# wgurecky/CORRLA_RS

Hardware: AMD Instinct MI355X
Metric: RSVD GFLOP/s on 16k x 16k f32 rank-128 (higher is better)
Workload: dtype f32

## Files before the change

corrla_rs_amd/_lib.py:

```python
import ctypes as C
import os

PKG = os.path.dirname(os.path.abspath(__file__))
LIB_PATH = os.environ.get("CORRLA_RSVD_LIB") or os.path.join(PKG, "lib", "libcorrla_rsvd.so")

i64, u64, u32, i32, dbl, flt = C.c_int64, C.c_uint64, C.c_uint32, C.c_int32, C.c_double, C.c_float
vp = C.c_void_p

OK, EINVAL, ENOMEM, EHIP, ECOMM, ENUMERIC, ENODEV = range(7)
OMEGA_ON_DEVICE = 0x1
PCA_CENTER_FUSED = 0x2
PCA_CENTER_COPY = 0x4
QR_HOUSEHOLDER = 0x8
SEED_EXPLICIT = 0x10
POWER_FUSED = 0x20
SHARD_COLS = 0x40
SKETCH_BF16X3 = 0x80
SKETCH_BF16X6 = 0x100
PCA_STANDARDIZE = 0x200
COV_CORRELATION = 0x1
COV_NO_CENTER = 0x2
COV_ROUTE_INPLACE, COV_ROUTE_INPLACE_CHECKED, COV_ROUTE_REPACKED = 1, 2, 3
COV_ROUTES = {COV_ROUTE_INPLACE: "inplace", COV_ROUTE_INPLACE_CHECKED: "inplace_checked", COV_ROUTE_REPACKED: "repacked"}
PCA_APPLY_OWN_MEANS = 0x400
PCA_APPLY_ROUTE_INPLACE, PCA_APPLY_ROUTE_INPLACE_CHECKED, PCA_APPLY_ROUTE_REPACKED = 1, 2, 3
PCA_APPLY_ROUTES = {PCA_APPLY_ROUTE_INPLACE: "inplace", PCA_APPLY_ROUTE_INPLACE_CHECKED: "inplace_checked",
                    PCA_APPLY_ROUTE_REPACKED: "repacked"}
PCA_APPLY_CENTRINGS = {1: "fused", 2: "copy"}
UNIQUE_ID_BYTES = 128


class Opts(C.Structure):
    _fields_ = [("struct_size", u32), ("flags", u32), ("seed", u64), ("omega", vp), ("omega_ld", i64),
                ("scales_out", vp)]


class Timings(C.Structure):
    _fields_ = [("total_ms", dbl), ("sketch_ms", dbl), ("power_ms", dbl), ("qr_ms", dbl), ("project_ms", dbl),
                ("small_svd_ms", dbl), ("finalize_ms", dbl), ("qr_passes", i32), ("n_collectives", i32),
                ("sketch_kernel_ms", dbl), ("host_enqueue_ms", dbl), ("collective_bytes", dbl), ("n_mixed_products", i32),
                ("n_bf16_products", i32), ("knn_ms", dbl), ("fit_ms", dbl)]


def _sigs():
    s = {
        "corrla_version": (C.c_char_p, []),
        "corrla_last_error": (C.c_char_p, []),
        "corrla_device_count": (C.c_int, []),
        "corrla_ctx_create": (C.c_int, [C.c_int, C.POINTER(vp)]),
        "corrla_ctx_destroy": (None, [vp]),
        "corrla_ctx_synchronize": (C.c_int, [vp]),
        "corrla_ctx_get_timings": (C.c_int, [vp, C.POINTER(Timings)]),
        "corrla_ctx_set_phase_timings": (C.c_int, [vp, C.c_int]),
        "corrla_ctx_comm_info": (C.c_int, [vp, C.POINTER(C.c_int), C.POINTER(C.c_int)]),
        "corrla_comm_unique_id": (C.c_int, [vp]),
        "corrla_ctx_comm_init": (C.c_int, [vp, vp, C.c_int, C.c_int]),
        "corrla_ctx_last_pca_apply": (C.c_int, [vp, C.POINTER(C.c_int), C.POINTER(C.c_int)]),
    }
    for suf, sc in (("f32", flt), ("f64", dbl)):
        rsvd = [vp, vp, i64, i64, i64, i64, i64, i64, i64, C.POINTER(Opts), vp, i64, vp, vp, i64]
        s["corrla_rsvd_" + suf] = (C.c_int, rsvd)
        s["corrla_rsvd_dev_" + suf] = (C.c_int, rsvd)
        s["corrla_rsvd_sharded_dev_" + suf] = (C.c_int, rsvd)
        pca = [vp, vp, i64, i64, i64, i64, i64, i64, i64, C.POINTER(Opts), vp, vp, vp, i64]
        s["corrla_pca_" + suf] = (C.c_int, pca)
        s["corrla_pca_dev_" + suf] = (C.c_int, pca)
        s["corrla_pca_sharded_dev_" + suf] = (C.c_int, pca)
        pw = [vp, vp, i64, i64, i64, i64, i64, i64, C.POINTER(Opts), vp, i64]
        s["corrla_power_iter_" + suf] = (C.c_int, pw)
        s["corrla_power_iter_dev_" + suf] = (C.c_int, pw)
        s["corrla_matmul_dev_" + suf] = (C.c_int, [vp, C.c_int, vp, i64, i64, i64, i64, vp, i64, i64, sc, vp, i64])
        rsvd_csr = [vp, vp, vp, vp, i64, i64, i64, i64, i64, i64, C.POINTER(Opts), vp, i64, vp, vp, i64]
        s["corrla_rsvd_csr_" + suf] = (C.c_int, rsvd_csr)
        s["corrla_rsvd_csr_dev_" + suf] = (C.c_int, rsvd_csr)
        pca_csr = [vp, vp, vp, vp, i64, i64, i64, i64, i64, i64, C.POINTER(Opts), vp, vp, vp, i64]
        s["corrla_pca_csr_" + suf] = (C.c_int, pca_csr)
        s["corrla_pca_csr_dev_" + suf] = (C.c_int, pca_csr)
        s["corrla_spmm_csr_dev_" + suf] = (C.c_int, [vp, C.c_int, vp, vp, vp, i64, i64, i64, vp, i64, i64, sc, vp, i64])
        cov = [vp, vp, i64, i64, i64, i64, u64, C.c_int, vp, vp, vp, i64, C.POINTER(C.c_int)]
        s["corrla_cov_" + suf] = (C.c_int, cov)
        s["corrla_cov_dev_" + suf] = (C.c_int, cov)
        model = [vp, vp, vp, i64, i64, u64, vp, i64, vp, vp]
        s["corrla_pca_transform_" + suf] = s["corrla_pca_transform_dev_" + suf] = (C.c_int, [vp, vp, i64, i64, i64, i64] + model)
        s["corrla_pca_transform_csr_" + suf] = s["corrla_pca_transform_csr_dev_" + suf] = (C.c_int, [vp, vp, vp, vp, i64, i64, i64] + model)
        inverse = [vp, vp, i64, i64, i64, vp, vp, vp, i64, i64, vp, i64]
        s["corrla_pca_inverse_" + suf] = s["corrla_pca_inverse_dev_" + suf] = (C.c_int, inverse)
        points = [vp, vp, i64, i64, vp, i64, i64, i64, C.c_int, dbl]
        s["corrla_rbf_matrix_" + suf] = s["corrla_rbf_matrix_dev_" + suf] = (C.c_int, points + [vp, i64])
        s["corrla_rbf_apply_" + suf] = s["corrla_rbf_apply_dev_" + suf] = (C.c_int, points + [C.c_int, vp, i64, i64, vp, i64])
        s["corrla_fill_normal_dev_" + suf] =(C.c_int, [vp, vp, i64, i64, i64, i64, u64, i64, i64])
        s["corrla_time_sketch_dev_" + suf] = (C.c_int, [vp, vp, i64, i64, i64, i64, vp, i64, i64, vp, i64, C.c_int,
                                                         C.POINTER(dbl)])
    s["corrla_rsvd_bf16"] = s["corrla_rsvd_dev_bf16"] = s["corrla_rsvd_f32"]
    s["corrla_pca_bf16"] = s["corrla_pca_dev_bf16"] = s["corrla_pca_f32"]
    s["corrla_matmul_dev_bf16"] = s["corrla_matmul_dev_f32"]
    grad = [vp, vp, i64, i64, vp, vp, i64, C.c_int, i64, dbl, vp, i64, C.POINTER(C.c_int)]
    s["corrla_grad_mat_f64"] = (C.c_int, grad)
    s["corrla_grad_mat_dev_f64"] = (C.c_int, grad)
    return s


SIGNATURES = _sigs()
_lib = None


class CorrlaError(RuntimeError):
    def __init__(self, code, msg):
        super().__init__(f"corrla_rsvd error {code}: {msg}")
        self.code = code


def load():
    global _lib
    if _lib is not None:
        return _lib
    if not os.path.exists(LIB_PATH):
        raise ImportError(
            f"{LIB_PATH} is missing: build it with `python -m corrla_rs_amd.build` (hipcc, gfx950). "
            "corrla_rs_amd has no CPU fallback.")
    try:
        import torch
    except ImportError:
        pass
    lib = C.CDLL(LIB_PATH, mode=C.RTLD_GLOBAL)
    for name, (res, args) in SIGNATURES.items():
        fn = getattr(lib, name)
        fn.restype = res
        fn.argtypes = args
    _lib = lib
    return lib


def check(code):
    if code != OK:
        msg = load().corrla_last_error().decode("utf-8", "replace")
        if code == EINVAL:
            raise ValueError(f"corrla_rsvd: {msg}")
        if code == ENOMEM:
            raise MemoryError(f"corrla_rsvd: {msg}")
        raise CorrlaError(code, msg)
```

corrla_rs_amd/api.py:

```python
import atexit
import ctypes as C
import sys
import threading
import weakref

import numpy as np

from . import _lib as L

__all__ = ["Context", "default_context", "rsvd", "random_svd", "power_iter", "rpca", "PcaRsvd", "algorithmic_flops"]


def _is_torch(x):
    return type(x).__module__.split(".")[0] == "torch"


def _is_torch_csr(x):
    return _is_torch(x) and str(getattr(x, "layout", "")) == "torch.sparse_csr"


def _is_sparse(x):
    if isinstance(x, tuple):
        def nd(v):
            return v.ndim if hasattr(v, "ndim") else np.ndim(v)
# ... 549 lines not shown
        if on_dev:
            import torch
            out = torch.empty((n_q, n_s), dtype=xq.dtype, device=xq.device)
            _sync_stream(xq)
        else:
            out = np.empty((n_q, n_s), dtype=xq.dtype)
        L.check(self._entry("corrla_rbf_matrix_", on_dev, xq.dtype)(self._h, _ptr(xq), n_q, self._row_stride(xq), _ptr(xs), n_s,
                                                                   self._row_stride(xs), dim, self._rbf_kernel_id(kernel_type),
                                                                   float(kernel_param), _ptr(out), n_s))
        if on_dev:
            L.check(self._lib.corrla_ctx_synchronize(self._h))
        return out

    def rbf_apply(self, x_query, x_support, coeffs, kernel_type, kernel_param=0.0, *, poly_degree=None):
        xq, xs, on_dev = self._rbf_points(x_query, x_support, "rbf_apply")
        n_q, dim = (int(v) for v in xq.shape)
        n_s = int(xs.shape[0])
        if poly_degree is not None and (isinstance(poly_degree, (bool, np.bool_)) or not isinstance(poly_degree, (int, np.integer))):
            raise ValueError("poly_degree must be None or an integer")
        degree = -1 if poly_degree is None or poly_degree < 0 else int(poly_degree)
        n_poly = 0 if degree < 0 else (dim + 1 if degree < 2 else dim + dim * (dim + 1) // 2 + 1)
        _reject_bf16(coeffs, "rbf_apply")
        if _is_sparse(coeffs):
            raise ValueError("rbf_apply takes dense coefficients")
        w = self._model_array(coeffs, xq, on_dev)
        if w.ndim == 1:
            w = w.reshape(-1, 1)
        if w.ndim != 2 or w.shape[1] == 0:
            raise ValueError("coeffs must be a non-empty matrix")
        if w.shape[0] != n_s + n_poly:
            raise ValueError(f"coeffs must have n_s + n_poly = {n_s} + {n_poly} rows, got {w.shape[0]}")
        w = self._rbf_rowmajor(w, on_dev)
        n_rhs = int(w.shape[1])
        if on_dev:
            import torch
            out = torch.empty((n_q, n_rhs), dtype=xq.dtype, device=xq.device)
            _sync_stream(xq)
        else:
            out = np.empty((n_q, n_rhs), dtype=xq.dtype)
        L.check(self._entry("corrla_rbf_apply_", on_dev, xq.dtype)(self._h, _ptr(xq), n_q, self._row_stride(xq), _ptr(xs), n_s,
                                                                  self._row_stride(xs), dim, self._rbf_kernel_id(kernel_type),
                                                                  float(kernel_param), degree, _ptr(w), self._row_stride(w), n_rhs,
                                                                  _ptr(out), n_rhs))
        if on_dev:
            L.check(self._lib.corrla_ctx_synchronize(self._h))
        return out

    def _run_product(self, name, operand, m, n, xt, trans, beta, in_dtype=None):
        import torch
        xin, xout = (m, n) if trans else (n, m)
        l = xt.shape[1]
        xc = xt.t().contiguous()
        res = torch.empty((l, xout), dtype=xt.dtype, device=xt.device)
        _sync_stream(xt)
        L.check(self._entry(name, True, in_dtype or xt.dtype)(self._h, 1 if trans else 0, *_c_args(operand), xc.data_ptr(), xin, l, float(beta),
                                                  res.data_ptr(), xout))
        return res.t()

    def spmm(self, a_csr, x, trans=False, beta=1.0):
        import torch
        vals, ci, rp, (m, n), on_dev = _as_csr(a_csr)
        dev = torch.device(f"cuda:{self.device}")
        if not on_dev:
            vals, ci, rp = (torch.from_numpy(v).to(dev) for v in (vals, ci, rp))
        xt = x if _is_torch(x) else torch.as_tensor(np.asarray(x))
        xt = xt.to(device=dev, dtype=vals.dtype)
        if xt.dim() != 2 or xt.shape[0] != (m if trans else n):
            raise ValueError(f"x must have {m if trans else n} rows")
        return self._run_product("corrla_spmm_csr_", (vals, ci, rp, m, n, int(vals.shape[0])),
                                 m, n, xt, trans, beta)

    def matmul(self, a, x, trans=False, beta=1.0):
        m, n = a.shape
        if _is_bf16(x):
            raise ValueError("matmul: x must be float32 or float64 (only the matrix a may be bfloat16)")
        if _is_bf16(a):
            if not str(x.dtype).endswith("float32"):
                raise ValueError("matmul: a bfloat16 a takes a float32 x")
            assert x.shape[0] == (m if trans else n)
            return self._run_product("corrla_matmul_", (a, m, n, *a.stride()), m, n, x, trans, beta, in_dtype=a.dtype)
        assert x.shape[0] == (m if trans else n) and x.dtype == a.dtype
        return self._run_product("corrla_matmul_", (a, m, n, *a.stride()), m, n, x, trans, beta)

    def grad_mat(self, x_mat, y, est_order, n_nbrs, x_query=None, *, scale=1.0):
        est_order, n_nbrs = int(est_order), int(n_nbrs)
        nreg = C.c_int(0)
        if _is_torch(x_mat) and x_mat.is_cuda:
            import torch
            x = x_mat.to(torch.float64).contiguous()
            yv = (y if _is_torch(y) else torch.as_tensor(np.asarray(y))).to(device=x.device, dtype=torch.float64).reshape(-1).contiguous()
            xq = x if x_query is None else x_query.to(device=x.device, dtype=torch.float64).contiguous()
            if x.dim() != 2 or xq.dim() != 2 or xq.shape[1] != x.shape[1] or yv.numel() != x.shape[0]:
                raise ValueError("x_mat (n, k), y (n,), x_query (n_q, k) expected")
            g = torch.empty((xq.shape[0], x.shape[1]), dtype=torch.float64, device=x.device)
            _sync_stream(x)
            L.check(self._lib.corrla_grad_mat_dev_f64(self._h, x.data_ptr(), x.shape[0], x.shape[1], yv.data_ptr(), xq.data_ptr(),
                                                      xq.shape[0], est_order, n_nbrs, float(scale), g.data_ptr(), x.shape[1],
                                                      C.byref(nreg)))
            return g.t(), nreg.value
        x = np.ascontiguousarray(np.asarray(x_mat, dtype=np.float64))
        yv = np.ascontiguousarray(np.asarray(y, dtype=np.float64).reshape(-1))
        xq = x if x_query is None else np.ascontiguousarray(np.asarray(x_query, dtype=np.float64))
        if x.ndim != 2 or xq.ndim != 2 or xq.shape[1] != x.shape[1] or yv.size != x.shape[0]:
            raise ValueError("x_mat (n, k), y (n,), x_query (n_q, k) expected")
        g = np.empty((xq.shape[0], x.shape[1]), dtype=np.float64)
        L.check(self._lib.corrla_grad_mat_f64(self._h, x.ctypes.data, x.shape[0], x.shape[1], yv.ctypes.data, xq.ctypes.data,
                                              xq.shape[0], est_order, n_nbrs, float(scale), g.ctypes.data, x.shape[1],
                                              C.byref(nreg)))
        return g.T, nreg.value

    def power_iter(self, a_mat, omega_rank, n_iter, *, seed=None, omega=None, qr=None):
        _reject_bf16(a_mat, "power_iter")
        a = np.asarray(a_mat)
        if a.ndim != 2:
            raise ValueError("a_mat must be 2-D")
        if a.dtype != np.float32:
            a = a.astype(np.float64, copy=False)
        m, n = a.shape
        w = int(omega_rank)
        rs, cs = _strides(a)
        o, keep = self._opts(seed, omega, n, w, a.dtype, False, self._qr_flag(qr))
        q = _empty_colmajor(a, m, max(w, 1))
        fn = self._entry("corrla_power_iter_", False, a.dtype)
        L.check(fn(self._h, a.ctypes.data, m, n, rs, cs, w, int(n_iter), C.byref(o) if o is not None else None,
                   q.ctypes.data, m))
        del keep
        return q

    def fill_normal(self, t, seed, row0=0, global_cols=None):
        rows, cols = t.shape
        rs, cs = t.stride()
        _sync_stream(t)
        fn = self._entry("corrla_fill_normal_", True, t.dtype)
        L.check(fn(self._h, t.data_ptr(), rows, cols, rs, cs, int(seed), int(row0),
                   int(global_cols if global_cols is not None else cols)))
        return t

    def time_sketch(self, a, x, reps=10):
        import torch
        m, n = a.shape
        rs, cs = a.stride()
        l = x.shape[1]
        xc = x.t().contiguous()
        y = torch.empty((l, m), dtype=a.dtype, device=a.device)
        ms = C.c_double()
        _sync_stream(a)
        fn = self._entry("corrla_time_sketch_", True, a.dtype)
        L.check(fn(self._h, a.data_ptr(), m, n, rs, cs, xc.data_ptr(), n, l, y.data_ptr(), m, int(reps), C.byref(ms)))
        return ms.value, y.t()


_default = None
_default_lock = threading.Lock()


def default_context():
    global _default
    with _default_lock:
        if _default is None:
            _default = Context(0)
        return _default


def rsvd(a_mat, n_rank, n_iters, n_oversamples, *, seed=None, omega=None, ctx=None, qr=None):
    return (ctx or default_context()).rsvd(a_mat, n_rank, n_iters, n_oversamples, seed=seed, omega=omega, qr=qr)

# ... 87 lines not shown
```

corrla_rs_amd/csrc/capi_impl.hpp:

```cpp
#pragma once
#include <cstddef>
#include <cstdint>
#include <cstring>
#include <string>
#include <vector>

#include "../../include/corrla_rsvd.h"
#include "driver.hpp"
#include "rbf_plan.hpp"

namespace corrla {

inline std::string& last_error_slot() {
  static thread_local std::string msg;
  return msg;
}

template <class F>
inline corrla_status guarded(F&& f) {
  try {
    f();
    return CORRLA_OK;
  } catch (const Error& e) {
    last_error_slot() = e.what();
// ... 368 lines not shown
    if (scales_out) dev.copy_values_out(sd.p, c.n, scales_out, c.host_ptrs);
  });
  finish_call(drv, dev, c.tm_out, false);
}

template <class Dev, class T>
inline void pca_entry(Dev& dev, bool host_ptrs, const T* x, int64_t m, int64_t n, int64_t rs, int64_t cs, int64_t rank,
                      int64_t n_iter, int64_t n_oversamples, const corrla_opts* opts, T* means, T* s, T* comps,
                      int64_t ldc, Timings* tm_out, bool profile, bool sharded = false) {
  PcaCall<T> c{host_ptrs, m, n, rank, n_iter, n_oversamples, opts, means, s, comps, ldc, tm_out, profile};
  c.sharded = sharded;
  pca_body(
      dev, c,
      [&] {
        validate_matrix(x, m, n, rs, cs);
        if (sharded) {
          if (rank < 1 || rank > n) throw Error(ST_EINVAL, "rank must be in [1, n_dim] for the sample-sharded PCA");
          if (n_iter < 0 || n_oversamples < 0) throw Error(ST_EINVAL, "n_iter and n_oversamples must be >= 0");
        } else {
          validate_rank(m, n, rank, n_iter, n_oversamples);
        }
      },
      [&] { return stage_input<Dev, T>(dev, host_ptrs, x, m, n, rs, cs, sharded); });
}

template <class Dev, class T>
inline void power_iter_entry(Dev& dev, bool host_ptrs, const T* a, int64_t m, int64_t n, int64_t rs, int64_t cs,
                             int64_t width, int64_t n_iter, const corrla_opts* opts, T* q, int64_t ldq) {
  if (!q) throw Error(ST_EINVAL, "q is NULL");
  validate_matrix(a, m, n, rs, cs);
  if (width < 1 || width > n) throw Error(ST_EINVAL, "width must be in [1, n]");
  if (n_iter < 0) throw Error(ST_EINVAL, "n_iter must be >= 0");
  if (ldq < m) throw Error(ST_EINVAL, "ldq < m");
  RunOpts ro = parse_opts(opts, !host_ptrs);
  if (ro.omega && ro.omega_ld < n) throw Error(ST_EINVAL, "omega_ld < n");
  if (!ro.seed_explicit && !ro.omega) ro.seed = dev.fresh_seed(false);
  dev.begin_call();
  TallA<T> ta = stage_input<Dev, T>(dev, host_ptrs, a, m, n, rs, cs, true);
  RsvdDriver<Dev, T> drv(dev, false);
  Skinny<T> y = dev.template alloc_skinny<T>(ta.mt, width);
  Skinny<T> y2 = dev.template alloc_skinny<T>(ta.mt, width);
  drv.power_iter(ta, width, n_iter, ro, y, y2);
  dev.copy_out(y, width, q, ldq, false, host_ptrs);
  dev.end_call();
}

template <class Dev, class T, class Validate, class Stage>
inline void product_body(Dev& dev, int trans, int64_t m, int64_t n, const T* x, int64_t ldx, int64_t l, T beta, T* res,
                         int64_t ldres, Timings* tm_out, Validate&& validate, Stage&& stage) {
  if (!x || !res) throw Error(ST_EINVAL, "x or res is NULL");
  validate();
  if (l < 1) throw Error(ST_EINVAL, "l must be >= 1");
  const int64_t xin = trans ? m : n, xout = trans ? n : m;
  if (ldx < xin || ldres < xout) throw Error(ST_EINVAL, "leading dimension too small");
  dev.begin_call();
  TallA<T> ta = stage();
  RsvdDriver<Dev, T> drv(dev, false);
  if (!ta.sparse) drv.mixed_planes_ = parse_opts(nullptr, true).mixed_planes;
  Skinny<T> xs = dev.template alloc_skinny<T>(xin, l);
  dev.copy_in_skinny(x, ldx, xs);
  Skinny<T> out = ta.sparse ? caller_skinny(res, xout, l, ldres) : dev.template alloc_skinny<T>(xout, l);
  T* beta_dev = dev.template alloc_scalar<T>(1);
  dev.store_values(&beta, (int64_t)1, beta_dev, false);
  if (trans)
    drv.at_times(ta, xs, out, beta_dev, false);
  else
    drv.a_times(ta, xs, out, beta_dev);
  if (!out.external) dev.copy_out(out, l, res, ldres, false, false);
  dev.end_call();
  if (tm_out) {
    tm_out->n_mixed_products = drv.tm.n_mixed_products;
    tm_out->n_bf16_products = drv.tm.n_bf16_products;
  }
}

template <class Dev, class T>
inline void matmul_entry(Dev& dev, int trans, const T* a, int64_t m, int64_t n, int64_t rs, int64_t cs, const T* x,
                         int64_t ldx, int64_t l, T beta, T* res, int64_t ldres, Timings* tm_out = nullptr) {
  product_body(
      dev, trans, m, n, x, ldx, l, beta, res, ldres, tm_out, [&] { validate_matrix(a, m, n, rs, cs); },
      [&] { return stage_input<Dev, T>(dev, false, a, m, n, rs, cs, true); });
}

inline void validate_csr_args(const void* values, const void* ci, const void* rp, int64_t m, int64_t n, int64_t nnz) {
  if (!values || !ci || !rp) throw Error(ST_EINVAL, "values, col_idx or row_ptr is NULL");
  if (m < 1 || n < 1) throw Error(ST_EINVAL, "matrix must have at least one row and one column");
  if (m > 0x7fffffff || n > 0x7fffffff) throw Error(ST_EINVAL, "CSR input: m and n must be below 2^31");
  if (nnz < 1) throw Error(ST_EINVAL, "CSR input: nnz must be >= 1");
  if (nnz > 0x7fffffff) throw Error(ST_EINVAL, "CSR input: nnz must be below 2^31");
}

template <class Dev, class T>
inline TallA<T> stage_csr(Dev& dev, bool host_ptrs, const T* values, const int32_t* ci, const int64_t* rp, int64_t m, int64_t n,
                          int64_t nnz, bool keep_orientation) {
  CsrView<T> a;
  a.rows = m;
  a.cols = n;
  a.nnz = nnz;
  if (host_ptrs) {
    if (rp[m] != nnz) throw Error(ST_EINVAL, "invalid CSR matrix: row_ptr[m] != nnz");
    T* dv = (T*)dev.alloc_bytes(sizeof(T) * (size_t)nnz);
    int32_t* dc = (int32_t*)dev.alloc_bytes(sizeof(int32_t) * (size_t)nnz);
    int64_t* dr = (int64_t*)dev.alloc_bytes(sizeof(int64_t) * (size_t)(m + 1));
    dev.h2d_bytes(dv, values, sizeof(T) * (size_t)nnz);
    dev.h2d_bytes(dc, ci, sizeof(int32_t) * (size_t)nnz);
    dev.h2d_bytes(dr, rp, sizeof(int64_t) * (size_t)(m + 1));
    a.val = dv;
    a.ci = dc;
    a.rp = dr;
  } else {
    a.val = values;
    a.ci = ci;
    a.rp = rp;
  }
  dev.csr_plan(a, true);
  CsrView<T> at = dev.csr_transpose(a);
  dev.csr_plan(at, false);
  TallA<T> ta;
  ta.sparse = true;
  const bool fat = !keep_orientation && m < n;
  ta.mt = fat ? n : m;
  ta.nt = fat ? m : n;
  ta.csr = fat ? at : a;
  ta.csr_t = fat ? a : at;
  return ta;
}

template <class Dev, class T>
inline void rsvd_csr_entry(Dev& dev, bool host_ptrs, const T* values, const int32_t* ci, const int64_t* rp, int64_t m, int64_t n,
                           int64_t nnz, int64_t rank, int64_t n_iter, int64_t n_oversamples, const corrla_opts* opts, T* u,
                           int64_t ldu, T* s, T* vt, int64_t ldvt, Timings* tm_out, bool profile) {
  static_assert(dev_has_spmm<Dev>::value, "CSR entries need a backend with SpMM kernels");
  RsvdCall<T> c{host_ptrs, m, rank, n_iter, n_oversamples, opts, u, ldu, s, vt, ldvt, tm_out, profile};
  c.sparse = true;
  c.fat = m < n;
  rsvd_body(
      dev, c,
      [&] {
        validate_csr_args(values, ci, rp, m, n, nnz);
        validate_rank(m, n, rank, n_iter, n_oversamples);
      },
      [&] { return stage_csr<Dev, T>(dev, host_ptrs, values, ci, rp, m, n, nnz, false); });
}

template <class Dev, class T>
inline void pca_csr_entry(Dev& dev, bool host_ptrs, const T* values, const int32_t* ci, const int64_t* rp, int64_t m, int64_t n,
                          int64_t nnz, int64_t rank, int64_t n_iter, int64_t n_oversamples, const corrla_opts* opts, T* means,
                          T* s, T* comps, int64_t ldc, Timings* tm_out, bool profile) {
  static_assert(dev_has_spmm<Dev>::value, "CSR entries need a backend with SpMM kernels");
  PcaCall<T> c{host_ptrs, m, n, rank, n_iter, n_oversamples, opts, means, s, comps, ldc, tm_out, profile};
  c.sparse = true;
  pca_body(
      dev, c,
      [&] {
        validate_csr_args(values, ci, rp, m, n, nnz);
        validate_rank(m, n, rank, n_iter, n_oversamples);
      },
      [&] { return stage_csr<Dev, T>(dev, host_ptrs, values, ci, rp, m, n, nnz, false); });
}

template <class Dev, class T>
inline void spmm_entry(Dev& dev, int trans, const T* values, const int32_t* ci, const int64_t* rp, int64_t m, int64_t n, int64_t nnz,
                       const T* x, int64_t ldx, int64_t l, T beta, T* res, int64_t ldres) {
  static_assert(dev_has_spmm<Dev>::value, "CSR entries need a backend with SpMM kernels");
  product_body(
      dev, trans, m, n, x, ldx, l, beta, res, ldres, (Timings*)nullptr, [&] { validate_csr_args(values, ci, rp, m, n, nnz); },
// ... 276 lines not shown
```

corrla_rs_amd/csrc/corrla_rsvd.hip:

```cpp
#include <mutex>
#include <vector>

#include "capi_impl.hpp"
#include "core_svd_stage.hpp"
#include "cov_stage.hpp"
#include "grad_stage.hpp"
#include "hip_backend.hpp"
#include "pca_apply_stage.hpp"
#include "rbf_stage.hpp"
#include "tall_stage.hpp"

using namespace corrla;

struct corrla_ctx {
  HipDev dev;
  Timings last;
  std::mutex mu;
  bool profile;
  pca_apply_stage::Ran pca_apply;
  explicit corrla_ctx(int ordinal) : dev(ordinal), profile(env_int("CORRLA_PROFILE_PHASES", 0) != 0) {}
};

namespace {
inline corrla_ctx* need(corrla_ctx* c) {
  if (!c) throw Error(ST_EINVAL, "ctx is NULL");
  return c;
}
template <class F>
inline void locked_call(corrla_ctx* c, F&& f) {
  std::lock_guard<std::mutex> lk(c->mu);
  try {
    f();
  } catch (...) {
    (void)hipSetDevice(c->dev.device);
    if (c->dev.stream) (void)hipStreamSynchronize(c->dev.stream);
    (void)hipGetLastError();
    throw;
  }
}

template <class F, class After>
inline corrla_status ctx_call(corrla_ctx* ctx, F&& f, After&& after) {
  return guarded([&] {
    corrla_ctx* c = need(ctx);
    locked_call(c, [&] { f(*c); });
    after(*c);
  });
}
template <class F>
inline corrla_status ctx_call(corrla_ctx* ctx, F&& f) {
  return ctx_call(ctx, f, [](corrla_ctx&) {});
}
inline void debug_qr_breakdown(const corrla_ctx& c) {
  if (c.profile && env_int("CORRLA_DEBUG", 0))
    std::fprintf(stderr, "[corrla] qr breakdown (ms): gram %.3f  download+check %.3f  host chol/inv %.3f  upload+apply %.3f  (%d passes)\n",
                 c.last.qr_gram_ms, c.last.qr_down_ms, c.last.qr_host_ms, c.last.qr_apply_ms, c.last.qr_passes);
}
template <class T>
corrla_status fill_c(corrla_ctx* ctx, T* p, int64_t rows, int64_t cols, int64_t rs, int64_t cs, uint64_t seed,
                     int64_t row0, int64_t global_cols) {
  return guarded([&] {
    corrla_ctx* c = need(ctx);
    if (!p) throw Error(ST_EINVAL, "p is NULL");
    if (rows < 0 || cols < 0 || rs < 0 || cs < 0 || global_cols < cols) throw Error(ST_EINVAL, "bad fill_normal shape");
    std::lock_guard<std::mutex> lk(c->mu);
    CORRLA_HIP(hipSetDevice(c->dev.device));
    c->dev.fill_normal(p, rows, cols, rs, cs, seed, row0, global_cols);
    c->dev.sync();
  });
}
template <class T>
corrla_status time_sketch_c(corrla_ctx* ctx, const T* a, int64_t m, int64_t n, int64_t rs, int64_t cs, const T* x,
                            int64_t ldx, int64_t l, T* y, int64_t ldy, int reps, double* avg_ms) {
  return guarded([&] {
    corrla_ctx* c = need(ctx);
    if (!x || !y || !avg_ms) throw Error(ST_EINVAL, "NULL argument");
    if (reps < 1 || l < 1 || ldx < n || ldy < m) throw Error(ST_EINVAL, "bad time_sketch arguments");
    std::lock_guard<std::mutex> lk(c->mu);
    HipDev& dev = c->dev;
    dev.begin_call();
    TallA<T> ta = stage_input<HipDev, T>(dev, false, a, m, n, rs, cs, true);
    RsvdDriver<HipDev, T> drv(dev, false);
    drv.mixed_planes_ = parse_opts(nullptr, true).mixed_planes;
    Skinny<T> xs = dev.alloc_skinny<T>(n, l);
    dev.copy_in_skinny(x, ldx, xs);
    Skinny<T> out = dev.alloc_skinny<T>(m, l);
    *avg_ms = dev.time_on_stream(reps, [&] { drv.a_times(ta, xs, out, nullptr); });
    dev.copy_out(out, l, y, ldy, false, false);
    dev.end_call();
  });
}
}

// ... 156 lines not shown
      pca_bf16_entry<HipDev>(c.dev, HOST, x, m, n, rs, cs, rank, n_iter, p, o, means, s, comps, ldc, &c.last, c.profile); \
    });                                                                                                                 \
  }
CORRLA_DEFINE_RSVD_BF16(corrla_rsvd_bf16, true)
CORRLA_DEFINE_RSVD_BF16(corrla_rsvd_dev_bf16, false)
CORRLA_DEFINE_PCA_BF16(corrla_pca_bf16, true)
CORRLA_DEFINE_PCA_BF16(corrla_pca_dev_bf16, false)
CORRLA_API corrla_status corrla_matmul_dev_bf16(corrla_ctx* ctx, int trans, CORRLA_DENSE(uint16_t, a), CORRLA_PRODUCT_REST(float)) {
  return ctx_call(ctx, [&](corrla_ctx& c) {
    matmul_bf16_entry<HipDev>(c.dev, trans, a, m, n, rs, cs, x, ldx, l, beta, res, ldres, &c.last);
  });
}

#define CORRLA_DEFINE_COV(NAME, T, HOST)                                                                                \
  CORRLA_API corrla_status NAME(corrla_ctx* ctx, CORRLA_DENSE(T, x), uint64_t flags, int ddof, T* means_out, T* scales_out, \
                                T* c, int64_t ldc, int* route_out) {                                                    \
    return ctx_call(ctx, [&](corrla_ctx& cx) {                                                                          \
      cov_entry<HipDev, T>(cx.dev, x, m, n, rs, cs, flags, ddof, means_out, scales_out, c, ldc, route_out, [&] {        \
        cov_stage::run<T>(cx.dev, HOST, x, m, n, rs, cs, flags, ddof, means_out, scales_out, c, ldc, route_out);        \
      });                                                                                                               \
    });                                                                                                                 \
  }
CORRLA_DEFINE_COV(corrla_cov_f32, float, true)
CORRLA_DEFINE_COV(corrla_cov_f64, double, true)
CORRLA_DEFINE_COV(corrla_cov_dev_f32, float, false)
CORRLA_DEFINE_COV(corrla_cov_dev_f64, double, false)

#define CORRLA_PCA_MODEL(T) const T *means, const T *scales, const T *components, int64_t ldc, int64_t k, uint64_t flags, T *scores, \
                            int64_t ld_scores, T *resid_out, T *means_out
#define CORRLA_PCA_MODEL_CALL(T) PcaTransformCall<T>{m, n, means, scales, components, ldc, k, flags, scores, ld_scores, resid_out, means_out}
#define CORRLA_DEFINE_PCA_TRANSFORM(NAME, T, HOST)                                                                      \
  CORRLA_API corrla_status NAME(corrla_ctx* ctx, CORRLA_DENSE(T, x), CORRLA_PCA_MODEL(T)) {                             \
    return ctx_call(ctx, [&](corrla_ctx& cx) {                                                                          \
      cx.pca_apply = pca_apply_stage::Ran();                                                                            \
      const PcaTransformCall<T> c = CORRLA_PCA_MODEL_CALL(T);                                                           \
      if (!x) throw Error(ST_EINVAL, "pca_transform: x is NULL");                                                       \
      if (m < 1 || n < 1) throw Error(ST_EINVAL, "pca_transform: m and n must be >= 1");                                \
      if (rs < 0 || cs < 0) throw Error(ST_EINVAL, "pca_transform: negative strides are not supported");                \
      const PcaApplyRange xr{x, (size_t)((m - 1) * rs + (n - 1) * cs + 1) * sizeof(T), "x"};                            \
      pca_transform_entry<HipDev, T>(cx.dev, c, false, &xr, 1,                                                          \
                                     [&] { pca_apply_stage::run_dense<T>(cx.dev, HOST, x, rs, cs, c, &cx.pca_apply); }); \
    });                                                                                                                 \
  }
#define CORRLA_DEFINE_PCA_TRANSFORM_CSR(NAME, T, HOST)                                                                  \
  CORRLA_API corrla_status NAME(corrla_ctx* ctx, CORRLA_CSR_A(T), CORRLA_PCA_MODEL(T)) {                                \
    return ctx_call(ctx, [&](corrla_ctx& cx) {                                                                          \
      cx.pca_apply = pca_apply_stage::Ran();                                                                            \
      const PcaTransformCall<T> c = CORRLA_PCA_MODEL_CALL(T);                                                           \
      validate_csr_args(values, col_idx, row_ptr, m, n, nnz);                                                           \
      const PcaApplyRange op[3] = {{values, (size_t)nnz * sizeof(T), "values"},                                         \
                                   {col_idx, (size_t)nnz * sizeof(int32_t), "col_idx"},                                 \
                                   {row_ptr, (size_t)(m + 1) * sizeof(int64_t), "row_ptr"}};                            \
      pca_transform_entry<HipDev, T>(cx.dev, c, true, op, 3, [&] {                                                      \
        pca_apply_stage::run_csr<T>(cx.dev, HOST, values, col_idx, row_ptr, nnz, c, &cx.pca_apply);                     \
      });                                                                                                               \
    });                                                                                                                 \
  }
#define CORRLA_DEFINE_PCA_INVERSE(NAME, T, HOST)                                                                        \
  CORRLA_API corrla_status NAME(corrla_ctx* ctx, const T* scores, int64_t m, int64_t k, int64_t ld_scores, const T* means, \
                                const T* scales, const T* components, int64_t ldc, int64_t n, T* out, int64_t row_stride_out) { \
    return ctx_call(ctx, [&](corrla_ctx& cx) {                                                                          \
      cx.pca_apply = pca_apply_stage::Ran();                                                                            \
      pca_inverse_entry<HipDev, T>(cx.dev, scores, m, k, ld_scores, means, scales, components, ldc, n, out, row_stride_out, [&] { \
        pca_apply_stage::run_inverse<T>(cx.dev, HOST, scores, m, k, ld_scores, means, scales, components, ldc, n, out,   \
                                        row_stride_out, &cx.pca_apply);                                                 \
      });                                                                                                               \
    });                                                                                                                 \
  }
#define CORRLA_DEFINE_PCA_APPLY(SUF, T)                                  \
  CORRLA_DEFINE_PCA_TRANSFORM(corrla_pca_transform_##SUF, T, true)       \
  CORRLA_DEFINE_PCA_TRANSFORM(corrla_pca_transform_dev_##SUF, T, false)  \
  CORRLA_DEFINE_PCA_TRANSFORM_CSR(corrla_pca_transform_csr_##SUF, T, true)      \
  CORRLA_DEFINE_PCA_TRANSFORM_CSR(corrla_pca_transform_csr_dev_##SUF, T, false) \
  CORRLA_DEFINE_PCA_INVERSE(corrla_pca_inverse_##SUF, T, true)           \
  CORRLA_DEFINE_PCA_INVERSE(corrla_pca_inverse_dev_##SUF, T, false)
CORRLA_DEFINE_PCA_APPLY(f32, float)
CORRLA_DEFINE_PCA_APPLY(f64, double)
CORRLA_API corrla_status corrla_ctx_last_pca_apply(corrla_ctx* ctx, int* centring_out, int* route_out) {
  return guarded([&] {
    corrla_ctx* c = need(ctx);
    std::lock_guard<std::mutex> lk(c->mu);
    if (centring_out) *centring_out = c->pca_apply.centring;
    if (route_out) *route_out = c->pca_apply.route;
  });
}

#define CORRLA_RBF_POINTS(T) const T *xq, int64_t n_q, int64_t ldq, const T *xs, int64_t n_s, int64_t lds, int64_t dim, int kernel, double eps
#define CORRLA_DEFINE_RBF(SUF, DEV, T, HOST)                                                                            \
  CORRLA_API corrla_status corrla_rbf_matrix_##DEV##SUF(corrla_ctx* ctx, CORRLA_RBF_POINTS(T), T* out, int64_t ld_out) { \
    return ctx_call(ctx, [&](corrla_ctx& cx) {                                                                          \
      const RbfCall<T> c{xq, n_q, ldq, xs, n_s, lds, dim, kernel, eps, -1, nullptr, 0, 0, out, ld_out};                 \
      rbf_matrix_entry<HipDev, T>(cx.dev, c, [&] { rbf_stage::run_matrix<T>(cx.dev, HOST, c); });                       \
    });                                                                                                                 \
  }                                                                                                                     \
  CORRLA_API corrla_status corrla_rbf_apply_##DEV##SUF(corrla_ctx* ctx, CORRLA_RBF_POINTS(T), int poly_degree, const T* coeffs, \
                                                       int64_t ldw, int64_t n_rhs, T* out, int64_t ld_out) {            \
    return ctx_call(ctx, [&](corrla_ctx& cx) {                                                                          \
      const RbfCall<T> c{xq, n_q, ldq, xs, n_s, lds, dim, kernel, eps, poly_degree, coeffs, ldw, n_rhs, out, ld_out};   \
      rbf_apply_entry<HipDev, T>(cx.dev, c, [&] { rbf_stage::run_apply<T>(cx.dev, HOST, c); });                         \
    });                                                                                                                 \
  }
CORRLA_DEFINE_RBF(f32, , float, true)
CORRLA_DEFINE_RBF(f64, , double, true)
CORRLA_DEFINE_RBF(f32, dev_, float, false)
CORRLA_DEFINE_RBF(f64, dev_, double, false)

static corrla_status grad_mat_c(corrla_ctx* ctx, bool host_ptrs, const double* x, int64_t n_pts, int64_t kf, const double* y,
                                const double* xq, int64_t n_q, int est_order, int64_t n_nbrs, double out_scale, double* g,
                                int64_t ldg, int* n_regularised) {
  return ctx_call(ctx, [&](corrla_ctx& c) {
    HipDev& dev = c.dev;
    if (!x || !y || !xq || !g) throw Error(ST_EINVAL, "NULL argument");
    if (n_pts < 1 || n_q < 1 || kf < 1) throw Error(ST_EINVAL, "empty point set");
    if (ldg < kf) throw Error(ST_EINVAL, "ldg < k");
    const GradPlan plan = grad_plan(n_pts, kf, n_q, est_order, n_nbrs, env_int("CORRLA_KNN", 0), env_int("CORRLA_FIT", 0),
                                    dev.num_cus, kGradWideBudgetBytes, env_int("CORRLA_KNN2_WGS_PER_CU", 1));
    if (plan.error) throw Error(ST_EINVAL, plan.error);
    dev.begin_call();
    auto dbl = [&](int64_t n) { return (double*)dev.alloc_bytes(sizeof(double) * (size_t)n); };
    auto staged = [&](const double* h, int64_t n) {
      if (!host_ptrs) return h;
      double* d = dbl(n);
      CORRLA_HIP(hipMemcpyAsync(d, h, sizeof(double) * (size_t)n, hipMemcpyHostToDevice, dev.stream));
      return (const double*)d;
    };
    const GradCall call{staged(x, n_pts * kf), staged(y, n_pts), staged(xq, n_q * kf), host_ptrs ? dbl(n_q * kf) : g,
                        host_ptrs ? kf : ldg, n_pts, kf, n_q, n_nbrs, est_order, out_scale,
                        (int*)dev.alloc_bytes(sizeof(int) * (size_t)(n_q * n_nbrs)), (int*)dev.alloc_bytes(sizeof(int) * (size_t)n_q),
                        env_int("CORRLA_KNN2_PROF", 0) != 0};
    grad_stage::run(dev, call, plan);
    std::vector<int> hs((size_t)n_q);
    CORRLA_HIP(hipMemcpyAsync(hs.data(), call.status, sizeof(int) * (size_t)n_q, hipMemcpyDeviceToHost, dev.stream));
    if (host_ptrs)
      CORRLA_HIP(hipMemcpy2DAsync(g, sizeof(double) * (size_t)ldg, call.g, sizeof(double) * (size_t)kf, sizeof(double) * (size_t)kf,
                                  (size_t)n_q, hipMemcpyDeviceToHost, dev.stream));
    dev.event_mark(2);
    dev.end_call();
    c.last = Timings();
    c.last.knn_ms = dev.event_elapsed_ms(0, 1);
    c.last.fit_ms = dev.event_elapsed_ms(1, 2);
    c.last.total_ms = c.last.knn_ms + c.last.fit_ms;
    int bad = 0;
    for (int v : hs) bad += v != 0;
    if (n_regularised) *n_regularised = bad;
  });
}
CORRLA_API corrla_status corrla_grad_mat_f64(corrla_ctx* ctx, const double* x, int64_t n_pts, int64_t k, const double* y,
                                             const double* xq, int64_t n_q, int est_order, int64_t n_nbrs, double out_scale,
                                             double* g, int64_t ldg, int* n_regularised) {
  return grad_mat_c(ctx, true, x, n_pts, k, y, xq, n_q, est_order, n_nbrs, out_scale, g, ldg, n_regularised);
}
CORRLA_API corrla_status corrla_grad_mat_dev_f64(corrla_ctx* ctx, const double* x, int64_t n_pts, int64_t k, const double* y,
                                                 const double* xq, int64_t n_q, int est_order, int64_t n_nbrs,
                                                 double out_scale, double* g, int64_t ldg, int* n_regularised) {
  return grad_mat_c(ctx, false, x, n_pts, k, y, xq, n_q, est_order, n_nbrs, out_scale, g, ldg, n_regularised);
}

CORRLA_API corrla_status corrla_comm_unique_id(void* out128) {
  return guarded([&] {
    if (!out128) throw Error(ST_EINVAL, "out128 is NULL");
    ncclUniqueId id;
    CORRLA_NCCL(ncclGetUniqueId(&id));
    std::memset(out128, 0, CORRLA_UNIQUE_ID_BYTES);
    std::memcpy(out128, &id, sizeof(id));
  });
}
// ... 11 lines not shown
```

corrla_rs_amd/csrc/driver.hpp:

```cpp
#pragma once
#include <cstdio>
#include <chrono>
#include <cmath>
#include <cstdint>
#include <cstring>
#include <limits>
#include <stdexcept>
#include <string>
#include <functional>
#include <type_traits>
#include <vector>

#include "gemm_plan.hpp"
#include "small_linalg.hpp"

namespace corrla {

struct Error : std::runtime_error {
  int code;
  Error(int c, const std::string& m) : std::runtime_error(m), code(c) {}
};
enum { ST_OK = 0, ST_EINVAL = 1, ST_ENOMEM = 2, ST_EHIP = 3, ST_ECOMM = 4, ST_ENUMERIC = 5, ST_ENODEV = 6 };

inline int64_t round_up(int64_t x, int64_t a) { return (x + a - 1) / a * a; }


template <class T>
struct Skinny {
  T* p = nullptr;
  int64_t rows = 0, cols = 0, ld = 0, cols_alloc = 0;
  bool external = false;
  Skinny view_cols(int64_t c) const {
    Skinny s = *this;
    s.cols = c;
    return s;
  }
};

template <class T>
struct Big {
  const T* p = nullptr;
  int64_t rows = 0, cols = 0, ld = 0, cols_readable = 0;
};

template <class T>
inline Big<T> as_rowmajor_transposed(const Skinny<T>& y, int64_t ncols) {
  Big<T> b;
  b.p = y.p;
  b.rows = ncols;
  b.cols = y.rows;
  b.ld = y.ld;
  b.cols_readable = y.ld;
  return b;
}

template <class T>
struct CsrView {
  const T* val = nullptr;
  const int32_t* ci = nullptr;
  const int64_t* rp = nullptr;
  int64_t rows = 0, cols = 0, nnz = 0;
  int64_t n_long = 0, n_chunks = 0;
  const int64_t* long_row = nullptr;
  const int64_t* long_base = nullptr;
  const int32_t* chunk_long = nullptr;
};

template <class D, class = void>
struct dev_has_spmm : std::false_type {};
template <class D>
struct dev_has_spmm<D, std::void_t<decltype(D::kHasSpmm)>> : std::true_type {};

template <class D, class = void>
struct dev_has_bf16in : std::false_type {};
template <class D>
struct dev_has_bf16in<D, std::void_t<decltype(D::kHasBf16In)>> : std::true_type {};

template <class D, class = void>
struct dev_has_colvar : std::false_type {};
template <class D>
struct dev_has_colvar<D, std::void_t<decltype(D::kHasColVar)>> : std::true_type {};

template <class D, class = void>
struct dev_has_syrk : std::false_type {};
template <class D>
struct dev_has_syrk<D, std::void_t<decltype(D::kHasSyrk)>> : std::true_type {};

template <class D, class = void>
struct dev_has_pca_apply : std::false_type {};
template <class D>
struct dev_has_pca_apply<D, std::void_t<decltype(D::kHasPcaApply)>> : std::true_type {};

template <class D, class = void>
struct dev_has_rbf : std::false_type {};
template <class D>
struct dev_has_rbf<D, std::void_t<decltype(D::kHasRbf)>> : std::true_type {};

template <class T>
struct TallA {
  Big<T> mem;
  bool row_major = true;
  int64_t mt = 0, nt = 0;
  const T* mu_short = nullptr;
  const T* mu_tall = nullptr;
  const T* inv_sd_short = nullptr;
  const T* inv_sd_tall = nullptr;
  bool sparse = false;
  CsrView<T> csr, csr_t;
  bool bf16 = false;
  Big<uint16_t> mem16;
};

struct RunOpts {
  uint64_t seed = 0x5eedull;
  bool seed_explicit = false;
  const void* omega = nullptr;
  int64_t omega_ld = 0;
  bool omega_on_device = false;
  bool sharded = false;
  int pca_center = 0;
  bool pca_standardize = false;
  bool qr_householder = false;
  bool power_fused = false;
  int mixed_planes = 0;
  bool mixed_project = true;
  int poison_core = 0;
};
constexpr int kFlagNonFinite = 2, kFlagNullCols = 4;

struct Timings {
  double total_ms = 0, sketch_ms = 0, power_ms = 0, qr_ms = 0, project_ms = 0, small_svd_ms = 0, finalize_ms = 0;
  double host_enqueue_ms = 0;
  int qr_passes = 0;
  int n_collectives = 0;
  double collective_bytes = 0;
  double knn_ms = 0, fit_ms = 0;
  int n_mixed_products = 0;
  int n_bf16_products = 0;
  double qr_gram_ms = 0, qr_down_ms = 0, qr_host_ms = 0, qr_apply_ms = 0;
  double sketch_kernel_ms = 0;
};

struct PhaseTimer {
  using clk = std::chrono::steady_clock;
  clk::time_point t0;
  PhaseTimer() : t0(clk::now()) {}
  double lap() {
    auto t1 = clk::now();
    double ms = std::chrono::duration<double, std::milli>(t1 - t0).count();
    t0 = t1;
    return ms;
  }
};

template <class Dev, class T>
struct RsvdDriver {
  Dev& dev;
  Timings tm;
  bool profile_phases;
  bool qr_householder = false;
  static constexpr const T* kNone = nullptr;

  explicit RsvdDriver(Dev& d, bool profile = false) : dev(d), profile_phases(profile) {}

  int mixed_planes_ = 0;
  void sparse_times(const CsrView<T>& s, const Skinny<T>& x, Skinny<T>& y, const T* scale_dev) {
    if constexpr (dev_has_spmm<Dev>::value)
      dev.spmm(s, x, y, scale_dev);
    else
      throw Error(ST_EINVAL, "this backend has no SpMM kernels: sparse operands are not supported");
  }
  void bf16_times(bool tn, const Big<uint16_t>& r, const Skinny<T>& x, Skinny<T>& y, const T* scale_dev) {
    if constexpr (dev_has_bf16in<Dev>::value && std::is_same<T, float>::value)
      dev.gemm_bf16a(tn, r, x, y, scale_dev), ++tm.n_bf16_products;
    else
      throw Error(ST_EINVAL, "this backend has no bf16-input kernels: bf16 operands are not supported");
  }
  Skinny<T> scale_ws_;
  void set_scale_workspace(const Skinny<T>& ws) { scale_ws_ = ws; }
// ... 85 lines not shown
    }
  };
  struct Attempt {
    bool defer = false;
    void* st_pool = nullptr;
    int st_slots = 0, st_used = 0;
    int* flags_pool = nullptr;
    int flags_cap = 0, flags_used = 0;
    std::vector<Pending> pending;
    bool dirty = false;
  } att_;
  void* status_record(int i) const { return (char*)att_.st_pool + (size_t)i * kStatusBytes; }
  int64_t m_local_ = 0, m_global_ = -1;
  int64_t m_local_override_ = -1;
  int64_t global_rows(bool sharded) {
    if (!sharded) return m_local_;
    if (m_global_ < 0) m_global_ = dev.allreduce_sum_host(m_local_);
    return m_global_;
  }

  int hh_short_shards_ = -1;
  bool householder_usable(const Skinny<T>& y, bool sharded) {
    if (!qr_householder) return false;
    if (!sharded) return y.rows >= y.cols;
    if (hh_short_shards_ < 0) hh_short_shards_ = (int)dev.allreduce_sum_host(m_local_ < y.cols ? 1 : 0);
    return hh_short_shards_ == 0;
  }
  void householder_panel(Skinny<T>& y, Skinny<T>& tmp, bool sharded) {
    const int64_t l = y.cols;
    auto h = dev.householder_up(y, tmp);
    if (!sharded) {
      dev.householder_down(h, y, tmp);
      return;
    }
    const int64_t np = dev.nranks(), rk = dev.rank();
    Skinny<T> stack = dev.template alloc_skinny<T>(np * l, l), t2 = dev.template alloc_skinny<T>(np * l, l);
    Skinny<T> rv, cv;
    rv.p = h.r_root();
    rv.rows = rv.cols = rv.ld = rv.cols_alloc = l;
    dev.copy_block(rv, 0, 0, l, l, stack, rk * l, 0);
    dev.allreduce(stack.p, (size_t)stack.ld * (size_t)stack.cols_alloc);
    dev.householder_thin_q(stack, t2);
    cv.p = (T*)dev.alloc_zeroed_bytes((size_t)l * (size_t)l * sizeof(T));
    cv.rows = cv.cols = cv.ld = cv.cols_alloc = l;
    dev.copy_block(stack, rk * l, 0, l, l, cv, 0, 0);
    dev.householder_down(h, y, tmp, (const T*)cv.p);
  }
  void householder_thin_q_any_width(Skinny<T>& y, Skinny<T>& tmp, bool sharded) {
    const int64_t l = y.cols, m = y.rows;
    int64_t wmax = dev.template householder_max_width<T>();
    if (const char* e = std::getenv("CORRLA_HH_BLOCK")) wmax = std::max<int64_t>(1, std::min<int64_t>(wmax, std::atoll(e)));
    if (l <= wmax) {
      householder_panel(y, tmp, sharded);
      return;
    }
    const int64_t nb = (l + wmax - 1) / wmax, w = (l + nb - 1) / nb;
    std::vector<double> th;
    for (int64_t c0 = 0; c0 < l; c0 += w) {
      const int64_t wb = std::min(w, l - c0);
      Skinny<T> yb = dev.template alloc_skinny<T>(m, wb), tb = dev.template alloc_skinny<T>(m, wb);
      Skinny<T> pb = dev.template alloc_skinny<T>(m, wb);
      dev.copy_block(y, 0, c0, m, wb, yb, 0, 0);
      for (int pass = 0; pass < 5; ++pass) {
        double overlap2 = 0.0;
        if (c0 > 0) {
          Skinny<T> t = dev.template alloc_skinny<T>(c0, wb);
          dev.gemm_nn(as_rowmajor_transposed(y, c0), yb, t, kNone);
          if (sharded) dev.allreduce(t.p, (size_t)t.ld * (size_t)t.cols_alloc);
          if (pass >= 1) {
            th.resize((size_t)(c0 * wb));
            dev.download_skinny(t, c0, wb, th.data());
            for (double v : th) overlap2 += v * v;
          }
          dev.gemm_tn(as_rowmajor_transposed(y, c0), t, pb, kNone);
          dev.sub_inplace(yb, pb);
        }
        householder_panel(yb, tb, sharded);
        if (c0 == 0 || (pass >= 1 && overlap2 <= 0.25)) break;
      }
      dev.copy_block(yb, 0, 0, m, wb, y, 0, c0);
    }
  }

  int64_t orthonormalize(Skinny<T>& y, Skinny<T>& tmp, bool sharded, bool rough = false) {
    const int64_t l = y.cols;
    if (householder_usable(y, sharded)) {
      PhaseTimer qt0;
      householder_thin_q_any_width(y, tmp, sharded);
      ++tm.qr_passes;
      subphase(tm.qr_gram_ms, qt0);
      return l;
    }
    int64_t r = orthonormalize_core(y, tmp, sharded, rough);
    if (r < l && !att_.defer && (sharded ? global_rows(true) : y.rows) >= l) r = complete_basis(y, r, sharded);
    return r;
  }

  int64_t complete_basis(Skinny<T>& y, int64_t r, bool sharded) {
    const int64_t l = y.cols, c = l - r, m = y.rows;
    Skinny<T> yc = dev.template alloc_skinny<T>(m, c);
    Skinny<T> pc = dev.template alloc_skinny<T>(m, c);
    Skinny<T> tc = dev.template alloc_skinny<T>(m, c);
    dev.fill_normal(yc.p, m, c, (int64_t)1, yc.ld, (uint64_t)(0x9e3779b97f4a7c15ull ^ (uint64_t)(131 * r + l)), (int64_t)0, c);
    if (r > 0) {
      for (int pass = 0; pass < 2; ++pass) {
        Skinny<T> t = dev.template alloc_skinny<T>(r, c);
        dev.gemm_nn(as_rowmajor_transposed(y, r), yc, t, kNone);
        if (sharded) dev.allreduce(t.p, (size_t)t.ld * (size_t)t.cols_alloc);
        dev.gemm_tn(as_rowmajor_transposed(y, r), t, pc, kNone);
        dev.sub_inplace(yc, pc);
      }
    }
    const int64_t rc = orthonormalize_core(yc, tc, sharded, false);
    dev.copy_cols(yc, y, r, rc);
    return r + rc;
  }

  template <class Factor>
  void cholqr_pass(Skinny<T>& y, Skinny<T>& tmp, Skinny<T>& gd, bool sharded, bool inplace, Factor&& factor) {
    const int64_t l = y.cols;
    Skinny<T> yv = y.view_cols(l);
    dev.gemm_nn(as_rowmajor_transposed(y, l), yv, gd, kNone);
    if (sharded) dev.allreduce(gd.p, (size_t)gd.ld * (size_t)gd.cols_alloc);
    const Skinny<T> md = factor(gd);
    if (inplace) {
      dev.apply_inplace(y, l, md);
    } else {
      dev.gemm_tn(as_rowmajor_transposed(y, l), md, tmp, kNone);
      std::swap(y.p, tmp.p);
    }
  }

  struct BlockSplit {
    int64_t n1 = 0, n2 = 0;
    T* minus_one = nullptr;
  };
  BlockSplit block_split(int64_t l) {
    BlockSplit s;
    s.n1 = round_up((l + 1) / 2, (int64_t)4);
    s.n2 = l - s.n1;
    s.minus_one = dev.template alloc_scalar<T>(1);
    dev.fill_const(s.minus_one, (int64_t)1, (T)-1);
    return s;
  }
  template <class Factor>
  void blocked_factor_inverse(const Skinny<T>& g, const BlockSplit& s, Skinny<T>& md, Factor&& factor) {
    const int64_t n1 = s.n1, n2 = s.n2;
    Skinny<T> g11 = dev.template alloc_skinny<T>(n1, n1), g12 = dev.template alloc_skinny<T>(n1, n2);
    Skinny<T> g22 = dev.template alloc_skinny<T>(n2, n2), x11 = dev.template alloc_skinny<T>(n1, n1);
    Skinny<T> x22 = dev.template alloc_skinny<T>(n2, n2), r12 = dev.template alloc_skinny<T>(n1, n2);
    Skinny<T> t22 = dev.template alloc_skinny<T>(n2, n2), t12 = dev.template alloc_skinny<T>(n1, n2);
    Skinny<T> x12 = dev.template alloc_skinny<T>(n1, n2);
    dev.copy_block(g, 0, 0, n1, n1, g11, 0, 0);
    dev.copy_block(g, 0, n1, n1, n2, g12, 0, 0);
    dev.copy_block(g, n1, n1, n2, n2, g22, 0, 0);
    factor(g11, n1, 0, x11);
    dev.gemm_nn(as_rowmajor_transposed(x11, n1), g12, r12, kNone);
    dev.gemm_nn(as_rowmajor_transposed(r12, n2), r12, t22, kNone);
    dev.sub_inplace(g22, t22);
    factor(g22, n2, 1, x22);
    dev.gemm_tn(as_rowmajor_transposed(r12, n2), x22, t12, kNone);
    dev.gemm_tn(as_rowmajor_transposed(x11, n1), t12, x12, s.minus_one);
    dev.copy_block(x11, 0, 0, n1, n1, md, 0, 0);
    dev.copy_block(x12, 0, 0, n1, n2, md, 0, n1);
    dev.copy_block(x22, 0, 0, n2, n2, md, n1, n1);
  }

  int64_t orthonormalize_device(Skinny<T>& y, Skinny<T>& tmp, bool sharded, bool rough, bool polish) {
    const int64_t l = y.cols;
    PhaseTimer qt0;
    const bool inplace = dev.qr_inplace_fits(l);
    const bool single = dev.template device_chol_fits<T>(l);
    const int level = std::max(2, std::min(dev.robust_passes(), kRobustPasses));
    const bool inloop = rough && !polish;
    const int npass_even = level;
    const int npass = inloop ? (level <= 2 ? 1 : npass_even - 1) : (polish ? (level <= 2 ? 1 : 3) : level);
    const int always = (polish || inloop) ? 1 : 2;
    int* need = att_.flags_pool + att_.flags_used;
    int* null_mask = dev.alloc_flags((int)l);
    int* need_blk = dev.alloc_flags(2);
    void* st_scratch = dev.alloc_zeroed_bytes((size_t)2 * npass * kStatusBytes);
    void* insp = single ? nullptr : dev.template alloc_inspect<T>();
    Skinny<T> gd = dev.template alloc_skinny<T>(l, l);
    Skinny<T> md = dev.template alloc_skinny<T>(l, l);
    const double eps0 = (double)std::numeric_limits<T>::epsilon();
    double shift_rel = eps0 * std::max({16.0, 0.25 * std::sqrt((double)std::max<int64_t>(y.rows, 1)), single ? 0.0 : 2.0 * (double)l});
    if (const char* e = std::getenv("CORRLA_QR_SHIFT_SCALE")) shift_rel *= std::atof(e);
    float nullx = 1.f;
    if (const char* e = std::getenv("CORRLA_QR_NULL_EXCESS")) nullx = (float)std::atof(e);
    const BlockSplit split = single ? BlockSplit{} : block_split(l);
    for (int pass = 0; pass < npass; ++pass) {
      const int gate = pass < always ? -1 : (inplace ? pass - 1 : always + ((pass - always) / 2) * 2 - 1);
      dev.set_run_if(gate < 0 ? nullptr : need + gate);
      const int shift_mode = polish ? 2 : (pass == 0 ? 1 : 0);
      const float nx = (!polish && pass >= 2) ? nullx : 0.f;
      const float need_ratio = (inloop && pass == 0) ? 1e-2f : 0.f;
      cholqr_pass(y, tmp, gd, sharded, inplace, [&](Skinny<T>& g) {
        if (single) {
          dev.chol_inv_robust(g, l, kPivotTol, (float)shift_rel, shift_mode, nx, md, st_scratch, pass, need + pass, null_mask, nullptr,
                              need_ratio);
          return md;
        }
        dev.gram_inspect(g, l, (float)shift_rel, shift_mode, insp);
        const void* shp = dev.template inspect_shift_ptr<T>(insp);
        blocked_factor_inverse(g, split, md, [&](const Skinny<T>& blk, int64_t n, int which, Skinny<T>& x) {
          dev.chol_inv_robust(blk, n, kPivotTol, 0.f, 2, nx, x, st_scratch, 2 * pass + which, need_blk + which,
                              null_mask + which * split.n1, shp, need_ratio);
        });
        dev.template combine_need<T>(need + pass, need_ratio > 0.f ? nullptr : insp, need_blk, need_blk + 1);
        return md;
      });
      if (pass + 1 < npass || inloop)
        dev.refill_null(y, l, null_mask, (uint64_t)(0x9e3779b97f4a7c15ull ^ (uint64_t)(977 * (att_.flags_used + pass) + l)));
      if (pass < always) ++tm.qr_passes;
    }
    dev.set_run_if(nullptr);
    att_.pending.push_back(Pending::robust_chol(always, npass, (inloop && npass > 1) ? -1 : att_.flags_used, st_scratch, single ? 1 : 2));
    att_.flags_used += npass;
    subphase(tm.qr_gram_ms, qt0);
    return l;
  }

  int64_t orthonormalize_core(Skinny<T>& y, Skinny<T>& tmp, bool sharded, bool rough, bool polish = false) {
    const int64_t l = y.cols;
    int64_t r = l;
    if (att_.defer && (sharded || y.rows >= l) && att_.flags_used + kRobustPasses <= att_.flags_cap &&
        dev.template device_qr_robust_fits<T>(l))
      return orthonormalize_device(y, tmp, sharded, rough, polish);
    const int rpp = dev.template device_chol_fits<T>(l) ? 1 : (dev.template device_chol_blocked_fits<T>(l) ? 2 : 0);
    if (rpp > 0) {
      PhaseTimer qt0;
      const int npass = rough ? 1 : 2, nrec = npass * rpp;
      Skinny<T> gd0 = dev.template alloc_skinny<T>(l, l);
      Skinny<T> md0 = rpp == 1 ? dev.template alloc_skinny<T>(l, l) : Skinny<T>{};
      const bool defer = att_.defer && att_.st_used + nrec <= att_.st_slots;
      void* st_dev = defer ? status_record(att_.st_used) : dev.alloc_bytes((size_t)2 * rpp * kStatusBytes);
      const BlockSplit split = rpp == 1 ? BlockSplit{} : block_split(l);
      for (int pass = 0; pass < npass; ++pass) {
        cholqr_pass(y, tmp, gd0, sharded, false, [&](Skinny<T>& g) {
          if (rpp == 1) {
            dev.chol_inv(g, l, kPivotTol, md0, st_dev, pass);
            return md0;
          }
          Skinny<T> md = dev.template alloc_skinny<T>(l, l);
          blocked_factor_inverse(g, split, md, [&](const Skinny<T>& blk, int64_t n, int which, Skinny<T>& x) {
            dev.chol_inv(blk, n, kPivotTol, x, st_dev, 2 * pass + which);
          });
          return md;
        });
        ++tm.qr_passes;
      }
      if (defer) {
        att_.pending.push_back(Pending::optimistic_chol(att_.st_used, npass, rpp, !rough));
        att_.st_used += nrec;
        subphase(tm.qr_gram_ms, qt0);
        return l;
      }
      int fail[4] = {0, 0, 0, 0};
      float min_ratio[4], dev_i[4];
      dev.read_chol_status(st_dev, nrec, fail, min_ratio, dev_i);
      subphase(tm.qr_gram_ms, qt0);
      bool ok = true;
      for (int i = 0; i < nrec; ++i) {
        if (fail[i] == 3) throw Error(ST_ENUMERIC, "non-finite Gram matrix in orthonormalisation");
        ok = ok && fail[i] == 0;
      }
      if (rpp == 1 && fail[0] == 2) return 0;
      for (int i = nrec - rpp; !rough && i < nrec; ++i) ok = ok && dev_i[i] <= 0.25f;
      if (ok) return l;
    }
    if (att_.defer) att_.dirty = true;
    const double eps = (double)std::numeric_limits<T>::epsilon();
    std::vector<double> g((size_t)l * l), mm((size_t)l * l), uu, ss, vv;
    Skinny<T> gd = dev.template alloc_skinny<T>(l, l);
    Skinny<T> md = dev.template alloc_skinny<T>(l, l);
    int fails = 0;
    bool series_next = false;
    const double series_max_e = sizeof(T) == 4 ? 1e-2 : 1e-4;
    for (int pass = 0; pass < 12; ++pass) {
      if (r == 0) break;
      Skinny<T> yv = y.view_cols(r);
      Skinny<T> gv = gd.view_cols(r);
      gv.rows = r;
      PhaseTimer qt;
      dev.gemm_nn(as_rowmajor_transposed(y, r), yv, gv, kNone);
      if (sharded) dev.allreduce(gd.p, (size_t)gd.ld * (size_t)gd.cols_alloc);
      subphase(tm.qr_gram_ms, qt);
      ++tm.qr_passes;
      if (series_next) {
        Skinny<T> mv = md.view_cols(r);
        mv.rows = r;
        dev.inv_sqrt_series(gv, r, mv);
        Skinny<T> out = tmp.view_cols(r);
        dev.gemm_tn(as_rowmajor_transposed(y, r), mv, out, kNone);
        if (r < l) dev.zero_cols(tmp, r, l);
        std::swap(y.p, tmp.p);
        subphase(tm.qr_apply_ms, qt);
        break;
      }
      dev.download_skinny(gv, r, r, g.data());
      double gmax = 0.0, dev_i = 0.0;
      for (int64_t j = 0; j < r; ++j)
        for (int64_t i = 0; i < r; ++i) {
          const double x = g[(size_t)j * r + i];
          if (!std::isfinite(x)) throw Error(ST_ENUMERIC, "non-finite Gram matrix in orthonormalisation");
          dev_i = std::max(dev_i, std::fabs(x - (i == j ? 1.0 : 0.0)));
          if (i == j) gmax = std::max(gmax, x);
        }
      if (gmax == 0.0) {
        r = 0;
        break;
// ... 176 lines not shown
    long long clk, wall;
  };
  static_assert(sizeof(StatusRecord) == kStatusBytes, "status record layout");
  static void debug_record(int i, const char* what, const StatusRecord& r) {
    if (std::getenv("CORRLA_DEBUG"))
      std::fprintf(stderr, "[corrla] status record %d (%s): fail %d min_ratio %.3g dev_i %.3g\n", i, what, r.fail, r.min_ratio, r.dev_i);
  }
  Verdict attempt_verdict() {
    const Attempt& at = att_;
    if (at.dirty) return Verdict::kRepeatOnHost;
    if (at.pending.empty()) return Verdict::kClean;
    const size_t words_at = (size_t)at.st_slots * kStatusBytes;
    std::vector<char> host(words_at + (size_t)at.flags_used * sizeof(int));
    dev.read_bytes(at.st_pool, host.size(), host.data());
    std::vector<StatusRecord> rec((size_t)at.st_used);
    std::vector<int> flags((size_t)at.flags_used);
    if (!rec.empty()) std::memcpy(rec.data(), host.data(), rec.size() * sizeof(StatusRecord));
    if (!flags.empty()) std::memcpy(flags.data(), host.data() + words_at, flags.size() * sizeof(int));
    for (int f : flags)
      if (f & kFlagNonFinite) throw Error(ST_ENUMERIC, "non-finite Gram matrix in orthonormalisation");
    for (const Pending& p : at.pending) {
      for (int i = 0; p.kind == Pending::kOptimisticChol && i < p.npass * p.records_per_pass; ++i)
        if (rec[(size_t)(p.first_record + i)].fail == 3) throw Error(ST_ENUMERIC, "non-finite Gram matrix in orthonormalisation");
      if (p.kind == Pending::kCoreSvd && rec[(size_t)p.record].fail == 3) throw Error(ST_ENUMERIC, "non-finite core matrix in small SVD");
    }
    for (const Pending& p : at.pending) {
      const Verdict v = p.kind == Pending::kRobustChol ? judge_robust_chol(p, flags.data())
                        : p.kind == Pending::kCoreSvd  ? judge_core_svd(p, rec[(size_t)p.record])
                                                       : judge_optimistic_chol(p, &rec[(size_t)p.first_record]);
      if (v != Verdict::kClean) return v;
    }
    return Verdict::kClean;
  }
  Verdict judge_optimistic_chol(const Pending& p, const StatusRecord* r) {
    debug_record(p.first_record, "Cholesky", r[0]);
    const int nrec = p.npass * p.records_per_pass;
    for (int i = 0; i < nrec; ++i)
      if (r[i].fail != 0) return Verdict::kRepeatOnHost;
    for (int i = nrec - p.records_per_pass; p.verify_near_identity && i < nrec; ++i)
      if (!(r[i].dev_i <= 0.25f)) return Verdict::kRepeatOnHost;
    return Verdict::kClean;
  }
  Verdict judge_robust_chol(const Pending& p, const int* flags) {
    if (p.flag_slot < 0) return Verdict::kClean;
    const int* need = flags + p.flag_slot;
    for (int i = p.always; i < p.npass; ++i)
      if (need[i - 1] != 0) ++tm.qr_passes;
    if (std::getenv("CORRLA_DEBUG")) {
      std::fprintf(stderr, "[corrla] device thin-Q: %d passes enqueued, need_next =", p.npass);
      for (int i = 0; i < p.npass; ++i) std::fprintf(stderr, " %d", need[i]);
      const int nrec = p.npass * p.st_per_pass;
      std::vector<int> f2((size_t)nrec);
      std::vector<float> mr((size_t)nrec), di((size_t)nrec);
      dev.read_chol_status(p.st, nrec, f2.data(), mr.data(), di.data());
      std::fprintf(stderr, "; ||G - I||_max / min pivot ratio per factorisation:");
      for (int i = 0; i < nrec; ++i) std::fprintf(stderr, " %.2g/%.2g", di[(size_t)i], mr[(size_t)i]);
      std::fprintf(stderr, "\n");
    }
    return need[p.npass - 1] != 0 ? Verdict::kMorePasses : Verdict::kClean;
  }
  Verdict judge_core_svd(const Pending& p, const StatusRecord& r) {
    debug_record(p.record, "core SVD", r);
    if (r.fail == 0) dev.svd_sweeps_used((int)r.dev_i);
    if (r.fail == 1) return Verdict::kMoreSweeps;
    if (r.fail == 4) return Verdict::kNeedV;
    return r.fail == 0 ? Verdict::kClean : Verdict::kRepeatOnHost;
  }

  void random_svd_tall_body(const TallA<T>& a, int64_t k, int64_t l, int64_t n_iter, const RunOpts& o, Skinny<T>& u_tall,
                            T* s_dev, Skinny<T>& v_tall) {
    PhaseTimer total;
    const bool hh_tmp = qr_householder;
    Skinny<T> q = dev.template alloc_skinny_out<T>(a.mt, l);
    Skinny<T> q2 = hh_tmp ? dev.template alloc_skinny<T>(a.mt, l) : dev.template alloc_skinny_out<T>(a.mt, l);
    power_iter(a, l, n_iter, o, q, q2);
    PhaseTimer pt;
    Skinny<T> bt = dev.template alloc_skinny<T>(a.nt, l);
    mixed_planes_ = o.mixed_project ? o.mixed_planes : 0;
    at_times(a, q, bt, kNone, o.sharded);
    mixed_planes_ = 0;
    phase(tm.project_ms, pt);
    Skinny<T> qb = dev.template alloc_skinny<T>(a.nt, l);
    Skinny<T> qb2 = dev.template alloc_skinny<T>(a.nt, l);
    dev.copy_skinny(bt, qb);
    orthonormalize(qb, qb2, false);
    phase(tm.qr_ms, pt);
    Skinny<T> ct = dev.template alloc_skinny<T>(l, l);
    dev.gemm_nn(as_rowmajor_transposed(bt, l), qb, ct, kNone);
    if (o.poison_core) dev.poison_entry(ct, l / 2, l / 3, o.poison_core);
    Skinny<T> m1 = dev.template alloc_skinny<T>(l, k);
    Skinny<T> m2 = dev.template alloc_skinny<T>(l, k);
    void* svd_st = nullptr;
    if (att_.defer && att_.st_used + 1 <= att_.st_slots) {
      svd_st = status_record(att_.st_used);
      att_.pending.push_back(Pending::core_svd(att_.st_used));
      att_.st_used += 1;
    }
    dev.small_svd(ct, l, k, m2, m1, s_dev, svd_st);
    if (att_.defer) {
      Skinny<T> m1b = dev.template alloc_skinny<T>(l, k);
      orthonormalize_core(m1, m1b, false, true, true);
    }
    if (!att_.defer) {
      std::vector<T> sh((size_t)k);
      dev.copy_values_out(s_dev, k, sh.data(), true);
      const T null_tol = (T)(1e-3 * (double)std::numeric_limits<T>::epsilon()) * sh[0];
      int64_t nz = 0;
      while (nz < k && sh[(size_t)nz] > null_tol) ++nz;
      if (nz < k) complete_basis(m1, nz, false);
      if (nz == k) {
        Skinny<T> m1b = dev.template alloc_skinny<T>(l, k);
        orthonormalize_core(m1, m1b, false, true);
      }
    }
    phase(tm.small_svd_ms, pt);
    dev.gemm_tn(as_rowmajor_transposed(qb, l), m2, v_tall, kNone);
    dev.fix_signs(v_tall, m1, k);
    dev.gemm_tn(as_rowmajor_transposed(q, l), m1, u_tall, kNone);
    phase(tm.finalize_ms, pt);
    tm.host_enqueue_ms += total.lap();
  }

  void phase(double& slot, PhaseTimer& pt) {
    if (profile_phases) dev.sync();
    (void)pt.lap();
    dev.phase_mark(&slot);
  }
  void subphase(double& slot, PhaseTimer& pt) {
    if (!profile_phases) return;
    dev.sync();
    slot += pt.lap();
  }
};

template <class Dev, class T>
inline void small_svd_host(Dev& dev, const Skinny<T>& cd, int64_t l, int64_t k, Skinny<T>& m1, Skinny<T>& m2, T* s_dev) {
  std::vector<double> c((size_t)l * l), uc((size_t)l * l), vc((size_t)l * l), sv(l);
  dev.download_skinny(cd, l, l, c.data());
  const double eps = (double)std::numeric_limits<T>::epsilon();
  if (small::jacobi_svd((int)l, c.data(), (int)l, uc.data(), sv.data(), vc.data(), std::max(1e-15, eps * 1e-3)) < 0)
    throw Error(ST_ENUMERIC, "non-finite core matrix in small SVD");
  dev.upload_skinny(vc.data(), l, k, l, m1);
  dev.upload_skinny(uc.data(), l, k, l, m2);
  std::vector<T> st(k);
  for (int64_t i = 0; i < k; ++i) st[i] = (T)sv[i];
  dev.store_values(st.data(), k, s_dev, false);
}

struct Layout {
  bool fat;
  bool row_major;
  bool needs_pack;
  int64_t mt, nt, ld;
};

inline void validate_matrix(const void* a, int64_t m, int64_t n, int64_t rs, int64_t cs) {
  if (!a) throw Error(ST_EINVAL, "a is NULL");
  if (m < 1 || n < 1) throw Error(ST_EINVAL, "matrix must have at least one row and one column");
  if (rs < 0 || cs < 0) throw Error(ST_EINVAL, "negative strides are not supported");
  if (m > 1 && rs == 0) throw Error(ST_EINVAL, "row_stride == 0 with more than one row");
  if (n > 1 && cs == 0) throw Error(ST_EINVAL, "col_stride == 0 with more than one column");
}

inline Layout classify(int64_t m, int64_t n, int64_t rs, int64_t cs, bool force_tall) {
  Layout L;
  L.fat = !force_tall && m < n;
  L.mt = L.fat ? n : m;
  L.nt = L.fat ? m : n;
  const int64_t trs = L.fat ? cs : rs, tcs = L.fat ? rs : cs;
  L.needs_pack = false;
  if ((tcs == 1 || L.nt == 1) && (trs >= L.nt || L.mt == 1)) {
    L.row_major = true;
    L.ld = L.mt == 1 ? L.nt : trs;
  } else if ((trs == 1 || L.mt == 1) && (tcs >= L.mt || L.nt == 1)) {
    L.row_major = false;
    L.ld = L.nt == 1 ? L.mt : tcs;
  } else {
    L.row_major = true;
    L.needs_pack = true;
    L.ld = L.nt;
  }
  return L;
}

inline void validate_rank(int64_t m, int64_t n, int64_t rank, int64_t n_iter, int64_t n_oversamples) {
  if (rank < 1) throw Error(ST_EINVAL, "rank must be >= 1");
  if (n_iter < 0 || n_oversamples < 0) throw Error(ST_EINVAL, "n_iter and n_oversamples must be >= 0");
  if (rank > std::min(m, n)) throw Error(ST_EINVAL, "rank exceeds min(m, n) (the reference panics here)");
  if (rank + n_oversamples > (int64_t)1 << 20) throw Error(ST_EINVAL, "rank + n_oversamples too large");
}

}
```

corrla_rs_amd/csrc/hip_backend.hpp:

```cpp
#pragma once
#include <hip/hip_runtime.h>
#include <rccl/rccl.h>

#include <cmath>
#include <cstdio>
#include <cstdlib>
#include <cstring>
#include <limits>
#include <random>
#include <string>
#include <type_traits>
#include <utility>
#include <vector>

#include "core_svd_plan.hpp"
#include "driver.hpp"
#include "hip_kernels.hpp"
#include "tsqr_kernels.hpp"
#include "jacobi_mc_kernels.hpp"
#include "ata_kernels.hpp"
#include "tall_kernels.hpp"
#include "mixed_kernels.hpp"
#include "bf16in_kernels.hpp"
#include "grad_kernels.hpp"
#include "knn2_kernels.hpp"
#include "grad_wide_kernels.hpp"
#include "spmm_kernels.hpp"
#include "colvar_kernels.hpp"
#include "syrk_kernels.hpp"
#include "pca_apply_kernels.hpp"
#include "rbf_kernels.hpp"

namespace corrla {

#define CORRLA_HIP(call)                                                                                       \
  do {                                                                                                         \
    hipError_t e_ = (call);                                                                                    \
    if (e_ != hipSuccess)                                                                                      \
      throw Error(ST_EHIP, std::string(#call) + " failed: " + hipGetErrorString(e_) + " (" __FILE__ ":" +       \
                               std::to_string(__LINE__) + ")");                                                \
  } while (0)
#define CORRLA_NCCL(call)                                                                                      \
  do {                                                                                                         \
    ncclResult_t r_ = (call);                                                                                  \
    if (r_ != ncclSuccess) throw Error(ST_ECOMM, std::string(#call) + " failed: " + ncclGetErrorString(r_));   \
  } while (0)

inline int env_int(const char* name, int dflt) {
  const char* v = std::getenv(name);
  return v && *v ? std::atoi(v) : dflt;
}

template <class T>
struct NcclType;
template <>
struct NcclType<float> {
  static constexpr ncclDataType_t v = ncclFloat;
};
template <>
struct NcclType<double> {
  static constexpr ncclDataType_t v = ncclDouble;
};

template <int MAX, int N = 1, class F>
inline void with_nt(int n, const F& f) {
  if constexpr (N < MAX) {
    if (n > N) return with_nt<MAX, N + 1>(n, f);
  }
  if (n != N) throw Error(ST_EINVAL, "internal: no kernel instantiation for " + std::to_string(n));
  f(std::integral_constant<int, N>{});
}
template <int... Vs, class F>
inline void with_one_of(int n, const F& f) {
  if (!((n == Vs && (f(std::integral_constant<int, Vs>{}), true)) || ...))
    throw Error(ST_EINVAL, "internal: no kernel instantiation for " + std::to_string(n));
}
template <int... Vs, class F>
inline void with_one_of(std::integer_sequence<int, Vs...>, int n, const F& f) {
  with_one_of<Vs...>(n, f);
}
template <int MAX, int N = 1, class F>
inline void for_each_nt(const F& f) {
  f(std::integral_constant<int, N>{});
  if constexpr (N < MAX) for_each_nt<MAX, N + 1>(f);
}
template <int... Vs, class F>
inline void for_each_of(std::integer_sequence<int, Vs...>, const F& f) {
  (f(std::integral_constant<int, Vs>{}), ...);
}

inline void lds_limit(const void* fn, size_t bytes) {
  CORRLA_HIP(hipFuncSetAttribute(fn, hipFuncAttributeMaxDynamicSharedMemorySize, (int)bytes));
}
namespace core_svd_stage {
template <class T>
void set_lds_limits();
}
namespace tall_stage {
struct Call;
template <class T>
void set_lds_limits();
inline void set_lds_limits();
}
namespace rbf_stage {
template <class T>
void set_lds_limits();
}

class HipDev {
 public:
  int device = 0;
  int num_cus = 256;
  hipStream_t stream = nullptr;
  ncclComm_t comm = nullptr;
  int comm_rank = 0, comm_size = 1;
  int n_collectives = 0;
  double collective_bytes = 0;

  explicit HipDev(int dev_ordinal) : device(dev_ordinal) {
    int count = 0;
    if (hipGetDeviceCount(&count) != hipSuccess || count <= 0)
      throw Error(ST_ENODEV, "no HIP device visible (libcorrla_rsvd has no CPU fallback)");
    if (dev_ordinal < 0 || dev_ordinal >= count) throw Error(ST_EINVAL, "device ordinal out of range");
    CORRLA_HIP(hipSetDevice(device));
    hipDeviceProp_t prop;
    CORRLA_HIP(hipGetDeviceProperties(&prop, device));
    if (std::strncmp(prop.gcnArchName, "gfx950", 6) != 0)
      throw Error(ST_ENODEV, std::string("device is ") + prop.gcnArchName + ", this library is built for gfx950 only");
    num_cus = prop.multiProcessorCount;
    CORRLA_HIP(hipStreamCreateWithFlags(&stream, hipStreamNonBlocking));
    CORRLA_HIP(hipMalloc(&zero_page_, 256));
    CORRLA_HIP(hipHostMalloc(&pinned_, kPinnedBytes, hipHostMallocDefault));
    for (auto& e : events_) CORRLA_HIP(hipEventCreate(&e));
    CORRLA_HIP(hipMemsetAsync(zero_page_, 0, 256, stream));
    set_lds_limits();
    {
      std::random_device rd;
      entropy_ = ((uint64_t)rd() << 32) ^ (uint64_t)rd();
    }
    no_device_chol_ = env_int("CORRLA_HOST_CHOL", 0) != 0;
    robust_passes_ = std::max(2, env_int("CORRLA_ROBUST_PASSES", 2));
    robust_qr_ = env_int("CORRLA_DEVICE_ROBUST_QR", 1) != 0;
    gemm_debug_flags_ = env_int("CORRLA_GEMM_DEBUG", 0);
    gemm_knobs_.split_nn = env_int("CORRLA_SPLIT_NN", 0);
    gemm_knobs_.split_tn = env_int("CORRLA_SPLIT_TN", 0);
    gemm_knobs_.mw = env_int("CORRLA_MW", 0);
    gemm_knobs_.xcd_remap = env_int("CORRLA_GEMM_XCD", 1);
    gemm_knobs_.tall_min_rows = env_int("CORRLA_TALL_MIN_ROWS", 65536);
    gemm_knobs_.persist_max_tiles = env_int("CORRLA_GEMM_PERSIST_TILES", 16);
    gemm_knobs_.f64_waves = env_int("CORRLA_F64_WAVES", 8);
    if (const char* e = std::getenv("CORRLA_MIXED_MIN_WORK")) gemm_knobs_.mixed_min_work = std::atof(e);
    gemm_knobs_.even_blocks = env_int("CORRLA_EVEN_BLOCKS", 0) != 0;
    gemm_knobs_.no_gram_alias = env_int("CORRLA_NO_GRAM_ALIAS", 0) != 0;
    gemm_knobs_.no_rotate = env_int("CORRLA_GEMM_NO_ROTATE", 0) != 0;
    gemm_knobs_.mixed_split = env_int("CORRLA_MIXED_SPLIT", 0);
    syrk_knobs_.slab_rows = env_int("CORRLA_SYRK_SLAB_ROWS", 0);
  }
  ~HipDev() {
    (void)hipSetDevice(device);
    if (stream) (void)hipStreamSynchronize(stream);
    if (comm) (void)ncclCommDestroy(comm);
    for (auto& c : chunks_) (void)hipFree(c.p);
    for (auto& c : zchunks_) (void)hipFree(c.p);
    if (zero_page_) (void)hipFree(zero_page_);
    if (pinned_) (void)hipHostFree(pinned_);
    for (auto& e : events_)
      if (e) (void)hipEventDestroy(e);
    for (auto& e : ev_pool_) (void)hipEventDestroy(e);
    if (stream) (void)hipStreamDestroy(stream);
  }
  HipDev(const HipDev&) = delete;
  HipDev& operator=(const HipDev&) = delete;

  int nranks() const { return comm_size; }

  uint64_t fresh_seed(bool rank_invariant) {
    uint64_t z = (rank_invariant ? 0x5eedull : entropy_) + 0x9e3779b97f4a7c15ull * (uint64_t)(++(rank_invariant ? calls_sharded_ : calls_));
    z = (z ^ (z >> 30)) * 0xbf58476d1ce4e5b9ull;
    z = (z ^ (z >> 27)) * 0x94d049bb133111ebull;
    z ^= z >> 31;
    return z ? z : 0x5eedull;
  }

  void comm_init(const void* id128, int rank, int nranks_) {
    CORRLA_HIP(hipSetDevice(device));
    ncclUniqueId id;
    static_assert(sizeof(ncclUniqueId) <= CORRLA_UNIQUE_ID_BYTES, "unique id size");
    std::memcpy(&id, id128, sizeof(id));
    if (comm) {
      (void)ncclCommDestroy(comm);
      comm = nullptr;
    }
    CORRLA_NCCL(ncclCommInitRank(&comm, nranks_, id, rank));
    comm_rank = rank;
    comm_size = nranks_;
  }
  void comm_info(int* rank_out, int* nranks_out) {
    if (!comm) {
      *rank_out = 0;
      *nranks_out = 0;
      return;
    }
    CORRLA_NCCL(ncclCommUserRank(comm, rank_out));
    CORRLA_NCCL(ncclCommCount(comm, nranks_out));
  }

  void begin_call() {
    CORRLA_HIP(hipSetDevice(device));
    events_set_[0] = events_set_[1] = events_set_[2] = false;
    n_collectives = 0;
    collective_bytes = 0;
    marks_.clear();
    ev_used_ = 0;
    phase_mark(nullptr);
    for (auto& c : chunks_) c.used = 0;
    sp_scratch_ = nullptr;
    sp_scratch_bytes_ = 0;
    for (auto& c : zchunks_) {
      c.zeroed = std::min<size_t>(c.used, (size_t)256 << 20);
      c.used = 0;
      if (c.zeroed) CORRLA_HIP(hipMemsetAsync(c.p, 0, c.zeroed, stream));
    }
  }
  void end_call() { sync(); }
  void sync() { CORRLA_HIP(hipStreamSynchronize(stream)); }

  void* alloc_bytes(size_t bytes) {
    bytes = (bytes + 255) / 256 * 256;
    if (bytes == 0) bytes = 256;
    for (auto& c : chunks_)
      if (c.size - c.used >= bytes) {
        void* p = (char*)c.p + c.used;
        c.used += bytes;
        return p;
      }
    Chunk c;
    c.size = std::max<size_t>(bytes, (size_t)64 << 20);
    if (hipMalloc(&c.p, c.size) != hipSuccess) {
      (void)hipGetLastError();
      throw Error(ST_ENOMEM, "device allocation of " + std::to_string(c.size) + " bytes failed");
    }
    c.used = bytes;
    chunks_.push_back(c);
    return c.p;
  }
  void memset_zero(void* p, size_t bytes) { CORRLA_HIP(hipMemsetAsync(p, 0, bytes, stream)); }
  void* alloc_zeroed(size_t bytes) {
    bytes = (bytes + 255) / 256 * 256;
    if (bytes == 0) bytes = 256;
    Chunk* hit = nullptr;
    for (auto& c : zchunks_)
      if (c.size - c.used >= bytes) {
        hit = &c;
        break;
      }
    if (!hit) {
      Chunk c;
      c.size = std::max<size_t>(bytes, (size_t)128 << 20);
      if (hipMalloc(&c.p, c.size) != hipSuccess) {
        (void)hipGetLastError();
        throw Error(ST_ENOMEM, "device allocation of " + std::to_string(c.size) + " bytes failed");
      }
      zchunks_.push_back(c);
      hit = &zchunks_.back();
    }
    char* p = (char*)hit->p + hit->used;
    const size_t end = hit->used + bytes;
    if (end > hit->zeroed) {
      const size_t from = std::max(hit->used, hit->zeroed);
      CORRLA_HIP(hipMemsetAsync((char*)hit->p + from, 0, end - from, stream));
    }
    hit->used = end;
    return p;
  }

  template <class T>
  static Skinny<T> skinny_of(int64_t rows, int64_t cols) {
    const SkinnyLayout lay = skinny_layout(rows, cols);
    Skinny<T> s;
    s.rows = rows;
    s.cols = cols;
    s.ld = lay.ld;
    s.cols_alloc = lay.cols_alloc;
    return s;
  }
  template <class T>
  Skinny<T> alloc_skinny(int64_t rows, int64_t cols) {
    Skinny<T> s = skinny_of<T>(rows, cols);
    const size_t bytes = (size_t)s.ld * (size_t)s.cols_alloc * sizeof(T);
    s.p = (T*)alloc_zeroed(bytes);
    return s;
  }
  template <class T>
  Skinny<T> alloc_skinny_out(int64_t rows, int64_t cols) {
    Skinny<T> s = skinny_of<T>(rows, cols);
    const size_t bytes = (size_t)s.ld * (size_t)s.cols_alloc * sizeof(T);
    if (bytes < ((size_t)4 << 20)) {
      s.p = (T*)alloc_zeroed(bytes);
      return s;
    }
    s.p = (T*)alloc_bytes(bytes);
    if (s.ld > rows)
      CORRLA_HIP(hipMemset2DAsync(s.p + rows, (size_t)s.ld * sizeof(T), 0, (size_t)(s.ld - rows) * sizeof(T), (size_t)s.cols_alloc,
                                  stream));
    if (s.cols_alloc > cols) memset_zero(s.p + cols * s.ld, (size_t)(s.cols_alloc - cols) * s.ld * sizeof(T));
    return s;
  }
  double* alloc_f64(int n) {
    return (double*)alloc_zeroed(sizeof(double) * n);
  }
  template <class T>
  T* alloc_scalar(int n) {
    return (T*)alloc_zeroed(sizeof(T) * n);
  }

  void h2d_2d(void* dst, int64_t dpitch_e, const void* src, int64_t spitch_e, int64_t width_e, int64_t rows, size_t esz) {
    CORRLA_HIP(hipMemcpy2DAsync(dst, (size_t)dpitch_e * esz, src, (size_t)spitch_e * esz, (size_t)width_e * esz,
                                (size_t)rows, hipMemcpyHostToDevice, stream));
    sync();
  }
  template <class T>
  void h2d_2d(T* dst, int64_t dpitch_e, const T* src, int64_t spitch_e, int64_t width_e, int64_t rows) {
    h2d_2d((void*)dst, dpitch_e, (const void*)src, spitch_e, width_e, rows, sizeof(T));
  }

  template <class T>
  void gemm_nn(const Big<T>& r, const Skinny<T>& x, Skinny<T>& out, const T* scale_dev);
  template <class T>
  void gemm_tn(const Big<T>& r, const Skinny<T>& x, Skinny<T>& out, const T* scale_dev);

  static constexpr bool kHasSpmm = true;
  template <class T>
  void csr_plan(CsrView<T>& v, bool check_idx);
  template <class T>
  CsrView<T> csr_transpose(const CsrView<T>& a);
  template <class T>
  void spmm(const CsrView<T>& s, const Skinny<T>& x, Skinny<T>& y, const T* scale_dev);
  void* spmm_scratch(size_t bytes) {
    if (bytes > sp_scratch_bytes_) {
      sp_scratch_ = alloc_bytes(bytes);
      sp_scratch_bytes_ = bytes;
    }
    return sp_scratch_;
  }
  void h2d_bytes(void* dst, const void* src, size_t bytes) {
    CORRLA_HIP(hipMemcpyAsync(dst, src, bytes, hipMemcpyHostToDevice, stream));
    sync();
  }

  template <class T>
  bool mixed_fits(bool tn, const Big<T>& r, const Skinny<T>& x, const Skinny<T>& out) const;
  template <class T>
  void gemm_mixed(bool tn, const Big<T>& r, const Skinny<T>& x, Skinny<T>& out, const T* scale_dev, int np);

  static constexpr bool kHasBf16In = true;
  bool bf16a_fits(const Big<uint16_t>& r, int64_t l) const;
  void gemm_bf16a(bool tn, const Big<uint16_t>& r, const Skinny<float>& x, Skinny<float>& out, const float* scale_dev);
  void widen_bf16(const uint16_t* src, int64_t rows, int64_t cols, int64_t rs, int64_t cs, float* dst, int64_t ldd) {
    const int64_t tiles_c = (cols + 31) / 32, tiles_r = (rows + 31) / 32;
    if (tiles_c * tiles_r > 0x7fffffff) throw Error(ST_EINVAL, "problem too large for the launch grid");
    hipLaunchKernelGGL(k::widen_bf16_kernel, dim3((unsigned)(tiles_c * tiles_r)), dim3(256), 0, stream, src, rows, cols, rs, cs, dst, ldd,
                       tiles_c);
    CORRLA_HIP(hipGetLastError());
  }

  template <class T>
  bool ata_fused_fits(const Big<T>& a, int64_t l) const;
  template <class T>
  void ata_fused(const Big<T>& a, const Skinny<T>& x, Skinny<T>& z);

  template <class T>
  void allreduce(T* p, size_t count) {
    if (comm_size <= 1 && !(comm && env_int("CORRLA_FORCE_ALLREDUCE", 0))) return;
    if (!comm) throw Error(ST_ECOMM, "communicator not initialised");
    CORRLA_NCCL(ncclAllReduce(p, p, count, NcclType<T>::v, ncclSum, comm, stream));
    ++n_collectives;
    collective_bytes += (double)count * sizeof(T);
  }
  void allreduce_f64(double* p, size_t count) { allreduce<double>(p, count); }
  int64_t allreduce_sum_host(int64_t v) {
    if (comm_size <= 1) return v;
    if (!comm) throw Error(ST_ECOMM, "communicator not initialised");
    double* d = alloc_f64(1);
    double h = (double)v;
    CORRLA_HIP(hipMemcpyAsync(d, &h, sizeof(double), hipMemcpyHostToDevice, stream));
    CORRLA_NCCL(ncclAllReduce(d, d, 1, ncclDouble, ncclSum, comm, stream));
    ++n_collectives;
    collective_bytes += sizeof(double);
    CORRLA_HIP(hipMemcpyAsync(&h, d, sizeof(double), hipMemcpyDeviceToHost, stream));
    sync();
    return (int64_t)(h + 0.5);
  }

  template <class T>
  void download_skinny(const Skinny<T>& s, int64_t rows, int64_t cols, double* host) {
    const size_t n = (size_t)rows * cols;
    std::vector<T> heap;
    T* tmp = (T*)pinned_;
    if (n * sizeof(T) > kPinnedBytes) {
      heap.resize(n);
      tmp = heap.data();
    }
    CORRLA_HIP(hipMemcpy2DAsync(tmp, (size_t)rows * sizeof(T), s.p, (size_t)s.ld * sizeof(T), (size_t)rows * sizeof(T),
                                (size_t)cols, hipMemcpyDeviceToHost, stream));
    sync();
    for (size_t i = 0; i < n; ++i) host[i] = (double)tmp[i];
  }
  template <class T>
  void upload_skinny(const double* host, int64_t rows, int64_t cols, int64_t ld_host, Skinny<T>& dst) {
    const size_t n = (size_t)dst.ld * dst.cols_alloc;
    std::vector<T> heap;
    T* tmp = (T*)pinned_;
// ... 566 lines not shown
    }
    hipEvent_t e = ev_pool_[ev_used_++];
    CORRLA_HIP(hipEventRecord(e, stream));
    marks_.push_back({e, slot});
  }
  void phase_forget() {
    for (auto& m_ : marks_) m_.slot = nullptr;
  }
  void phase_resolve(double* total) {
    for (size_t i = 1; i < marks_.size(); ++i) {
      float ms = 0.f;
      if (hipEventElapsedTime(&ms, marks_[i - 1].ev, marks_[i].ev) != hipSuccess) {
        (void)hipGetLastError();
        continue;
      }
      if (marks_[i].slot) *marks_[i].slot += (double)ms;
    }
    if (total && marks_.size() >= 2) {
      float ms = 0.f;
      if (hipEventElapsedTime(&ms, marks_.front().ev, marks_.back().ev) == hipSuccess)
        *total = (double)ms;
      else
        (void)hipGetLastError();
    }
    marks_.clear();
  }

  void event_mark(int i) {
    CORRLA_HIP(hipEventRecord(events_[i], stream));
    events_set_[i] = true;
  }
  double event_elapsed_ms(int i, int j) {
    if (!events_set_[i] || !events_set_[j]) return 0.0;
    float ms = 0.f;
    if (hipEventElapsedTime(&ms, events_[i], events_[j]) != hipSuccess) {
      (void)hipGetLastError();
      return 0.0;
    }
    return (double)ms;
  }

  template <class F>
  double time_on_stream(int reps, F&& f) {
    hipEvent_t e0, e1;
    CORRLA_HIP(hipEventCreate(&e0));
    CORRLA_HIP(hipEventCreate(&e1));
    f();
    CORRLA_HIP(hipEventRecord(e0, stream));
    for (int i = 0; i < reps; ++i) f();
    CORRLA_HIP(hipEventRecord(e1, stream));
    CORRLA_HIP(hipEventSynchronize(e1));
    float ms = 0.f;
    CORRLA_HIP(hipEventElapsedTime(&ms, e0, e1));
    (void)hipEventDestroy(e0);
    (void)hipEventDestroy(e1);
    return (double)ms / reps;
  }

 private:
  struct Chunk {
    void* p = nullptr;
    size_t size = 0, used = 0;
    size_t zeroed = 0;
  };
  std::vector<Chunk> chunks_;
  std::vector<Chunk> zchunks_;
  void* sp_scratch_ = nullptr;
  size_t sp_scratch_bytes_ = 0;
  void* zero_page_ = nullptr;
  void* pinned_ = nullptr;
  hipEvent_t events_[3] = {nullptr, nullptr, nullptr};
  bool events_set_[3] = {false, false, false};
  struct PhaseMark {
    hipEvent_t ev;
    double* slot;
  };
  std::vector<hipEvent_t> ev_pool_;
  size_t ev_used_ = 0;
  std::vector<PhaseMark> marks_;
  static constexpr size_t kPinnedBytes = (size_t)8 << 20;
  int gemm_debug_flags_ = 0;
  GemmKnobs gemm_knobs_;
  SyrkKnobs syrk_knobs_;
  uint64_t entropy_ = 0, calls_ = 0, calls_sharded_ = 0;
  bool no_device_chol_ = false;
  const int* run_if_ = nullptr;
  bool phase_events_ = true;
  bool robust_qr_ = true;
  int robust_passes_ = 2;
  CoreSvdState svd_state_;

  static void check_grid(const dim3& g) {
    if (g.y > 65535u || g.z > 65535u) throw Error(ST_EINVAL, "problem too large for the launch grid");
  }

  static void set_lds_limits() {
    constexpr size_t kMax = k::kLdsMaxBytes;
    set_lds_limits_typed<float>();
    set_lds_limits_typed<double>();
    core_svd_stage::set_lds_limits<float>();
    core_svd_stage::set_lds_limits<double>();
    tall_stage::set_lds_limits();
    lds_limit((const void*)k::knn_kernel, kMax);
    lds_limit((const void*)k::knn_mfma_kernel<4, 4>, kMax);
    lds_limit((const void*)k::knn_mfma_kernel<4, 8>, kMax);
    lds_limit((const void*)k::knn_mfma_kernel<4, 16>, kMax);
    lds_limit((const void*)k::knn_mfma_kernel<2, 4>, kMax);
    lds_limit((const void*)k::knn_mfma_kernel<2, 8>, kMax);
    lds_limit((const void*)k::knn_mfma_kernel<2, 16>, kMax);
    lds_limit((const void*)k::knn2_kernel<1>, k::k2_lds_bytes(1));
    lds_limit((const void*)k::knn2_kernel<2>, k::k2_lds_bytes(2));
    lds_limit((const void*)k::grad_fit_kernel, kMax);
    lds_limit((const void*)k::grad_fit_lin_kernel<1>, kMax);
    lds_limit((const void*)k::grad_fit_lin_kernel<2>, kMax);
    lds_limit((const void*)k::grad_fit_lin_kernel<3>, kMax);
    lds_limit((const void*)k::grad_fit_lin_kernel<4>, kMax);
    lds_limit((const void*)k::grad_fit_lin_kernel<5>, kMax);
    lds_limit((const void*)k::knn_wide_kernel, k::ws_lds_bytes());
    lds_limit((const void*)k::grad_fit_wide_kernel, k::wf_lds_bytes());
  }
  template <class T>
  static void set_lds_limits_typed() {
    constexpr size_t kMax = k::kLdsMaxBytes;
    tall_stage::set_lds_limits<T>();
    rbf_stage::set_lds_limits<T>();
    lds_limit((const void*)k::syrk_kernel<T, true>, (size_t)k::syrk_lds_bytes((int)sizeof(T)));
    lds_limit((const void*)k::syrk_kernel<T, false>, (size_t)k::syrk_lds_bytes((int)sizeof(T)));
    lds_limit((const void*)k::hh_leaf_factor_kernel<T, false>, kMax);
    lds_limit((const void*)k::hh_tree_factor_kernel<T, false>, kMax);
    lds_limit((const void*)k::hh_tree_apply_kernel<T, false>, kMax);
    lds_limit((const void*)k::hh_leaf_apply_kernel<T, false>, kMax);
    lds_limit((const void*)k::hh_leaf_factor_kernel<T, true>, kMax);
    lds_limit((const void*)k::hh_tree_factor_kernel<T, true>, kMax);
    lds_limit((const void*)k::hh_tree_apply_kernel<T, true>, kMax);
    lds_limit((const void*)k::hh_leaf_apply_kernel<T, true>, kMax);
  }
  tall_stage::Call tall_call();
  template <class T>
  void launch_gemm(bool tn, const Big<T>& r, const Skinny<T>& x, Skinny<T>& out, const T* scale_dev);

  template <class T>
  void launch_copy_out(const T* src, int64_t lds_, int64_t rows, int64_t cols, T* dst, int64_t ldd, bool transpose) {
    const int64_t tiles_c = (cols + 31) / 32, tiles_r = (rows + 31) / 32;
    if (tiles_c * tiles_r > 0x7fffffff) throw Error(ST_EINVAL, "problem too large for the launch grid");
    dim3 grid((unsigned)(tiles_c * tiles_r));
    hipLaunchKernelGGL((k::copy_out_kernel<T>), grid, dim3(256), 0, stream, src, lds_, rows, cols, dst, ldd,
                       transpose ? 1 : 0, tiles_c);
    CORRLA_HIP(hipGetLastError());
  }
};

}
```

include/corrla_rsvd.h:

```cpp
#ifndef CORRLA_RSVD_H
#define CORRLA_RSVD_H

#include <stddef.h>
#include <stdint.h>

#ifdef __cplusplus
extern "C" {
#endif

#if defined(__GNUC__)
#define CORRLA_API __attribute__((visibility("default")))
#else
#define CORRLA_API
#endif

typedef struct corrla_ctx corrla_ctx;

typedef enum corrla_status {
  CORRLA_OK = 0,
  CORRLA_EINVAL = 1,
  CORRLA_ENOMEM = 2,
  CORRLA_EHIP = 3,
  CORRLA_ECOMM = 4,
  CORRLA_ENUMERIC = 5,
// ... 185 lines not shown
#define CORRLA_PCA_APPLY_OWN_MEANS 0x400ull
#define CORRLA_PCA_APPLY_ROUTE_INPLACE 1
#define CORRLA_PCA_APPLY_ROUTE_INPLACE_CHECKED 2
#define CORRLA_PCA_APPLY_ROUTE_REPACKED 3
CORRLA_API corrla_status corrla_pca_transform_f32(corrla_ctx* ctx, const float* x, int64_t m, int64_t n, int64_t row_stride,
                                                  int64_t col_stride, const float* means, const float* scales, const float* components,
                                                  int64_t ldc, int64_t k, uint64_t flags, float* scores, int64_t ld_scores, float* resid_out,
                                                  float* means_out);
CORRLA_API corrla_status corrla_pca_transform_f64(corrla_ctx* ctx, const double* x, int64_t m, int64_t n, int64_t row_stride,
                                                  int64_t col_stride, const double* means, const double* scales, const double* components,
                                                  int64_t ldc, int64_t k, uint64_t flags, double* scores, int64_t ld_scores, double* resid_out,
                                                  double* means_out);
CORRLA_API corrla_status corrla_pca_transform_dev_f32(corrla_ctx* ctx, const float* x, int64_t m, int64_t n, int64_t row_stride,
                                                      int64_t col_stride, const float* means, const float* scales, const float* components,
                                                      int64_t ldc, int64_t k, uint64_t flags, float* scores, int64_t ld_scores, float* resid_out,
                                                      float* means_out);
CORRLA_API corrla_status corrla_pca_transform_dev_f64(corrla_ctx* ctx, const double* x, int64_t m, int64_t n, int64_t row_stride,
                                                      int64_t col_stride, const double* means, const double* scales, const double* components,
                                                      int64_t ldc, int64_t k, uint64_t flags, double* scores, int64_t ld_scores, double* resid_out,
                                                      double* means_out);
CORRLA_API corrla_status corrla_pca_transform_csr_f32(corrla_ctx* ctx, const float* values, const int32_t* col_idx,
                                                      const int64_t* row_ptr, int64_t m, int64_t n, int64_t nnz, const float* means,
                                                      const float* scales, const float* components, int64_t ldc, int64_t k, uint64_t flags,
                                                      float* scores, int64_t ld_scores, float* resid_out, float* means_out);
CORRLA_API corrla_status corrla_pca_transform_csr_f64(corrla_ctx* ctx, const double* values, const int32_t* col_idx,
                                                      const int64_t* row_ptr, int64_t m, int64_t n, int64_t nnz, const double* means,
                                                      const double* scales, const double* components, int64_t ldc, int64_t k, uint64_t flags,
                                                      double* scores, int64_t ld_scores, double* resid_out, double* means_out);
CORRLA_API corrla_status corrla_pca_transform_csr_dev_f32(corrla_ctx* ctx, const float* values, const int32_t* col_idx,
                                                          const int64_t* row_ptr, int64_t m, int64_t n, int64_t nnz, const float* means,
                                                          const float* scales, const float* components, int64_t ldc, int64_t k, uint64_t flags,
                                                          float* scores, int64_t ld_scores, float* resid_out, float* means_out);
CORRLA_API corrla_status corrla_pca_transform_csr_dev_f64(corrla_ctx* ctx, const double* values, const int32_t* col_idx,
                                                          const int64_t* row_ptr, int64_t m, int64_t n, int64_t nnz, const double* means,
                                                          const double* scales, const double* components, int64_t ldc, int64_t k, uint64_t flags,
                                                          double* scores, int64_t ld_scores, double* resid_out, double* means_out);
CORRLA_API corrla_status corrla_pca_inverse_f32(corrla_ctx* ctx, const float* scores, int64_t m, int64_t k, int64_t ld_scores,
                                                const float* means, const float* scales, const float* components, int64_t ldc, int64_t n,
                                                float* out, int64_t row_stride_out);
CORRLA_API corrla_status corrla_pca_inverse_f64(corrla_ctx* ctx, const double* scores, int64_t m, int64_t k, int64_t ld_scores,
                                                const double* means, const double* scales, const double* components, int64_t ldc, int64_t n,
                                                double* out, int64_t row_stride_out);
CORRLA_API corrla_status corrla_pca_inverse_dev_f32(corrla_ctx* ctx, const float* scores, int64_t m, int64_t k, int64_t ld_scores,
                                                    const float* means, const float* scales, const float* components, int64_t ldc, int64_t n,
                                                    float* out, int64_t row_stride_out);
CORRLA_API corrla_status corrla_pca_inverse_dev_f64(corrla_ctx* ctx, const double* scores, int64_t m, int64_t k, int64_t ld_scores,
                                                    const double* means, const double* scales, const double* components, int64_t ldc, int64_t n,
                                                    double* out, int64_t row_stride_out);
CORRLA_API corrla_status corrla_ctx_last_pca_apply(corrla_ctx* ctx, int* centring_out, int* route_out);

CORRLA_API corrla_status corrla_rbf_matrix_f32(corrla_ctx* ctx, const float* xq, int64_t n_q, int64_t ldq, const float* xs, int64_t n_s,
                                               int64_t lds, int64_t dim, int kernel, double eps, float* out, int64_t ld_out);
CORRLA_API corrla_status corrla_rbf_matrix_f64(corrla_ctx* ctx, const double* xq, int64_t n_q, int64_t ldq, const double* xs, int64_t n_s,
                                               int64_t lds, int64_t dim, int kernel, double eps, double* out, int64_t ld_out);
CORRLA_API corrla_status corrla_rbf_matrix_dev_f32(corrla_ctx* ctx, const float* xq, int64_t n_q, int64_t ldq, const float* xs, int64_t n_s,
                                                   int64_t lds, int64_t dim, int kernel, double eps, float* out, int64_t ld_out);
CORRLA_API corrla_status corrla_rbf_matrix_dev_f64(corrla_ctx* ctx, const double* xq, int64_t n_q, int64_t ldq, const double* xs, int64_t n_s,
                                                   int64_t lds, int64_t dim, int kernel, double eps, double* out, int64_t ld_out);
CORRLA_API corrla_status corrla_rbf_apply_f32(corrla_ctx* ctx, const float* xq, int64_t n_q, int64_t ldq, const float* xs, int64_t n_s,
                                              int64_t lds, int64_t dim, int kernel, double eps, int poly_degree, const float* coeffs,
                                              int64_t ldw, int64_t n_rhs, float* out, int64_t ld_out);
CORRLA_API corrla_status corrla_rbf_apply_f64(corrla_ctx* ctx, const double* xq, int64_t n_q, int64_t ldq, const double* xs, int64_t n_s,
                                              int64_t lds, int64_t dim, int kernel, double eps, int poly_degree, const double* coeffs,
                                              int64_t ldw, int64_t n_rhs, double* out, int64_t ld_out);
CORRLA_API corrla_status corrla_rbf_apply_dev_f32(corrla_ctx* ctx, const float* xq, int64_t n_q, int64_t ldq, const float* xs, int64_t n_s,
                                                  int64_t lds, int64_t dim, int kernel, double eps, int poly_degree, const float* coeffs,
                                                  int64_t ldw, int64_t n_rhs, float* out, int64_t ld_out);
CORRLA_API corrla_status corrla_rbf_apply_dev_f64(corrla_ctx* ctx, const double* xq, int64_t n_q, int64_t ldq, const double* xs, int64_t n_s,
                                                  int64_t lds, int64_t dim, int kernel, double eps, int poly_degree, const double* coeffs,
                                                  int64_t ldw, int64_t n_rhs, double* out, int64_t ld_out);

CORRLA_API corrla_status corrla_fill_normal_dev_f32(corrla_ctx* ctx, float* p, int64_t rows, int64_t cols, int64_t row_stride,
                                         int64_t col_stride, uint64_t seed, int64_t row0, int64_t global_cols);
CORRLA_API corrla_status corrla_fill_normal_dev_f64(corrla_ctx* ctx, double* p, int64_t rows, int64_t cols, int64_t row_stride,
                                         int64_t col_stride, uint64_t seed, int64_t row0, int64_t global_cols);

CORRLA_API corrla_status corrla_grad_mat_f64(corrla_ctx* ctx, const double* x, int64_t n_pts, int64_t k, const double* y,
                                             const double* xq, int64_t n_q, int est_order, int64_t n_nbrs, double out_scale,
                                             double* g, int64_t ldg, int* n_regularised);
CORRLA_API corrla_status corrla_grad_mat_dev_f64(corrla_ctx* ctx, const double* x, int64_t n_pts, int64_t k, const double* y,
                                                 const double* xq, int64_t n_q, int est_order, int64_t n_nbrs,
                                                 double out_scale, double* g, int64_t ldg, int* n_regularised);

CORRLA_API corrla_status corrla_time_sketch_dev_f32(corrla_ctx* ctx, const float* a, int64_t m, int64_t n, int64_t row_stride,
                                         int64_t col_stride, const float* x, int64_t ldx, int64_t l, float* y,
                                         int64_t ldy, int reps, double* avg_ms);
CORRLA_API corrla_status corrla_time_sketch_dev_f64(corrla_ctx* ctx, const double* a, int64_t m, int64_t n, int64_t row_stride,
                                         int64_t col_stride, const double* x, int64_t ldx, int64_t l, double* y,
                                         int64_t ldy, int reps, double* avg_ms);

#define CORRLA_UNIQUE_ID_BYTES 128
CORRLA_API corrla_status corrla_comm_unique_id(void* out128);
CORRLA_API corrla_status corrla_ctx_comm_init(corrla_ctx* ctx, const void* unique_id128, int rank, int nranks);

CORRLA_API corrla_status corrla_rsvd_sharded_dev_f32(corrla_ctx* ctx, const float* a_local, int64_t m_local, int64_t n,
                                          int64_t row_stride, int64_t col_stride, int64_t rank, int64_t n_iter,
                                          int64_t n_oversamples, const corrla_opts* opts, float* u_local, int64_t ldu,
                                          float* s, float* vt, int64_t ldvt);
CORRLA_API corrla_status corrla_rsvd_sharded_dev_f64(corrla_ctx* ctx, const double* a_local, int64_t m_local, int64_t n,
                                          int64_t row_stride, int64_t col_stride, int64_t rank, int64_t n_iter,
                                          int64_t n_oversamples, const corrla_opts* opts, double* u_local, int64_t ldu,
                                          double* s, double* vt, int64_t ldvt);

#ifdef __cplusplus
}
#endif
#endif
```

integration/rust/src/lib.rs:

```rust
use faer::{Mat, MatRef};
use std::ffi::CStr;
use std::os::raw::{c_char, c_int, c_void};

#[repr(C)]
pub struct CorrlaOpts {
    pub struct_size: u32,
    pub flags: u32,
    pub seed: u64,
    pub omega: *const c_void,
    pub omega_ld: i64,
    pub scales_out: *mut c_void,
}
pub const CORRLA_OMEGA_ON_DEVICE: u32 = 0x1;
pub const CORRLA_PCA_CENTER_FUSED: u32 = 0x2;
pub const CORRLA_PCA_CENTER_COPY: u32 = 0x4;
pub const CORRLA_QR_HOUSEHOLDER: u32 = 0x8;
pub const CORRLA_SEED_EXPLICIT: u32 = 0x10;
pub const CORRLA_POWER_FUSED: u32 = 0x20;
pub const CORRLA_SHARD_COLS: u32 = 0x40;
pub const CORRLA_SKETCH_BF16X3: u32 = 0x80;
pub const CORRLA_SKETCH_BF16X6: u32 = 0x100;
pub const CORRLA_PCA_STANDARDIZE: u32 = 0x200;
pub const CORRLA_COV_CORRELATION: u64 = 0x1;
pub const CORRLA_COV_NO_CENTER: u64 = 0x2;
// ... 24 lines not shown
                      ldc: i64) -> c_int;
    fn corrla_grad_mat_f64(ctx: *mut c_void, x: *const f64, n_pts: i64, k: i64, y: *const f64, xq: *const f64,
                           n_q: i64, est_order: c_int, n_nbrs: i64, out_scale: f64, g: *mut f64, ldg: i64,
                           n_regularised: *mut c_int) -> c_int;
    pub fn corrla_rsvd_csr_f32(ctx: *mut c_void, values: *const f32, col_idx: *const i32, row_ptr: *const i64, m: i64,
                               n: i64, nnz: i64, rank: i64, n_iter: i64, n_over: i64, opts: *const CorrlaOpts,
                               u: *mut f32, ldu: i64, s: *mut f32, vt: *mut f32, ldvt: i64) -> c_int;
    pub fn corrla_pca_csr_f32(ctx: *mut c_void, values: *const f32, col_idx: *const i32, row_ptr: *const i64, m: i64,
                              n: i64, nnz: i64, rank: i64, n_iter: i64, n_over: i64, opts: *const CorrlaOpts,
                              means: *mut f32, s: *mut f32, comps: *mut f32, ldc: i64) -> c_int;
    pub fn corrla_rsvd_csr_dev_f32(ctx: *mut c_void, values: *const f32, col_idx: *const i32, row_ptr: *const i64, m: i64,
                               n: i64, nnz: i64, rank: i64, n_iter: i64, n_over: i64, opts: *const CorrlaOpts,
                               u: *mut f32, ldu: i64, s: *mut f32, vt: *mut f32, ldvt: i64) -> c_int;
    pub fn corrla_pca_csr_dev_f32(ctx: *mut c_void, values: *const f32, col_idx: *const i32, row_ptr: *const i64, m: i64,
                              n: i64, nnz: i64, rank: i64, n_iter: i64, n_over: i64, opts: *const CorrlaOpts,
                              means: *mut f32, s: *mut f32, comps: *mut f32, ldc: i64) -> c_int;
    pub fn corrla_spmm_csr_dev_f32(ctx: *mut c_void, trans: c_int, values: *const f32, col_idx: *const i32,
                                   row_ptr: *const i64, m: i64, n: i64, nnz: i64, x: *const f32, ldx: i64, l: i64,
                                   beta: f32, res: *mut f32, ldres: i64) -> c_int;
    pub fn corrla_rsvd_csr_f64(ctx: *mut c_void, values: *const f64, col_idx: *const i32, row_ptr: *const i64, m: i64,
                               n: i64, nnz: i64, rank: i64, n_iter: i64, n_over: i64, opts: *const CorrlaOpts,
                               u: *mut f64, ldu: i64, s: *mut f64, vt: *mut f64, ldvt: i64) -> c_int;
    pub fn corrla_pca_csr_f64(ctx: *mut c_void, values: *const f64, col_idx: *const i32, row_ptr: *const i64, m: i64,
                              n: i64, nnz: i64, rank: i64, n_iter: i64, n_over: i64, opts: *const CorrlaOpts,
                              means: *mut f64, s: *mut f64, comps: *mut f64, ldc: i64) -> c_int;
    pub fn corrla_rsvd_csr_dev_f64(ctx: *mut c_void, values: *const f64, col_idx: *const i32, row_ptr: *const i64, m: i64,
                               n: i64, nnz: i64, rank: i64, n_iter: i64, n_over: i64, opts: *const CorrlaOpts,
                               u: *mut f64, ldu: i64, s: *mut f64, vt: *mut f64, ldvt: i64) -> c_int;
    pub fn corrla_pca_csr_dev_f64(ctx: *mut c_void, values: *const f64, col_idx: *const i32, row_ptr: *const i64, m: i64,
                              n: i64, nnz: i64, rank: i64, n_iter: i64, n_over: i64, opts: *const CorrlaOpts,
                              means: *mut f64, s: *mut f64, comps: *mut f64, ldc: i64) -> c_int;
    pub fn corrla_spmm_csr_dev_f64(ctx: *mut c_void, trans: c_int, values: *const f64, col_idx: *const i32,
                                   row_ptr: *const i64, m: i64, n: i64, nnz: i64, x: *const f64, ldx: i64, l: i64,
                                   beta: f64, res: *mut f64, ldres: i64) -> c_int;
    pub fn corrla_cov_f64(ctx: *mut c_void, x: *const f64, m: i64, n: i64, rs: i64, cs: i64, flags: u64, ddof: c_int,
                          means_out: *mut f64, scales_out: *mut f64, c: *mut f64, ldc: i64, route_out: *mut c_int) -> c_int;
    pub fn corrla_cov_f32(ctx: *mut c_void, x: *const f32, m: i64, n: i64, rs: i64, cs: i64, flags: u64, ddof: c_int,
                          means_out: *mut f32, scales_out: *mut f32, c: *mut f32, ldc: i64, route_out: *mut c_int) -> c_int;
    pub fn corrla_cov_dev_f64(ctx: *mut c_void, x: *const f64, m: i64, n: i64, rs: i64, cs: i64, flags: u64, ddof: c_int,
                              means_out: *mut f64, scales_out: *mut f64, c: *mut f64, ldc: i64, route_out: *mut c_int) -> c_int;
    pub fn corrla_cov_dev_f32(ctx: *mut c_void, x: *const f32, m: i64, n: i64, rs: i64, cs: i64, flags: u64, ddof: c_int,
                              means_out: *mut f32, scales_out: *mut f32, c: *mut f32, ldc: i64, route_out: *mut c_int) -> c_int;
    pub fn corrla_pca_transform_f64(ctx: *mut c_void, x: *const f64, m: i64, n: i64, rs: i64, cs: i64, means: *const f64,
                                     scales: *const f64, components: *const f64, ldc: i64, k: i64, flags: u64,
                                     scores: *mut f64, ld_scores: i64, resid_out: *mut f64, means_out: *mut f64) -> c_int;
    pub fn corrla_pca_transform_f32(ctx: *mut c_void, x: *const f32, m: i64, n: i64, rs: i64, cs: i64, means: *const f32,
                                     scales: *const f32, components: *const f32, ldc: i64, k: i64, flags: u64,
                                     scores: *mut f32, ld_scores: i64, resid_out: *mut f32, means_out: *mut f32) -> c_int;
    pub fn corrla_pca_transform_dev_f64(ctx: *mut c_void, x: *const f64, m: i64, n: i64, rs: i64, cs: i64, means: *const f64,
                                     scales: *const f64, components: *const f64, ldc: i64, k: i64, flags: u64,
                                     scores: *mut f64, ld_scores: i64, resid_out: *mut f64, means_out: *mut f64) -> c_int;
    pub fn corrla_pca_transform_dev_f32(ctx: *mut c_void, x: *const f32, m: i64, n: i64, rs: i64, cs: i64, means: *const f32,
                                     scales: *const f32, components: *const f32, ldc: i64, k: i64, flags: u64,
                                     scores: *mut f32, ld_scores: i64, resid_out: *mut f32, means_out: *mut f32) -> c_int;
    pub fn corrla_pca_transform_csr_f64(ctx: *mut c_void, values: *const f64, col_idx: *const i32, row_ptr: *const i64,
                                         m: i64, n: i64, nnz: i64, means: *const f64, scales: *const f64,
                                         components: *const f64, ldc: i64, k: i64, flags: u64, scores: *mut f64,
                                         ld_scores: i64, resid_out: *mut f64, means_out: *mut f64) -> c_int;
    pub fn corrla_pca_transform_csr_f32(ctx: *mut c_void, values: *const f32, col_idx: *const i32, row_ptr: *const i64,
                                         m: i64, n: i64, nnz: i64, means: *const f32, scales: *const f32,
                                         components: *const f32, ldc: i64, k: i64, flags: u64, scores: *mut f32,
                                         ld_scores: i64, resid_out: *mut f32, means_out: *mut f32) -> c_int;
    pub fn corrla_pca_transform_csr_dev_f64(ctx: *mut c_void, values: *const f64, col_idx: *const i32, row_ptr: *const i64,
                                         m: i64, n: i64, nnz: i64, means: *const f64, scales: *const f64,
                                         components: *const f64, ldc: i64, k: i64, flags: u64, scores: *mut f64,
                                         ld_scores: i64, resid_out: *mut f64, means_out: *mut f64) -> c_int;
    pub fn corrla_pca_transform_csr_dev_f32(ctx: *mut c_void, values: *const f32, col_idx: *const i32, row_ptr: *const i64,
                                         m: i64, n: i64, nnz: i64, means: *const f32, scales: *const f32,
                                         components: *const f32, ldc: i64, k: i64, flags: u64, scores: *mut f32,
                                         ld_scores: i64, resid_out: *mut f32, means_out: *mut f32) -> c_int;
    pub fn corrla_pca_inverse_f64(ctx: *mut c_void, scores: *const f64, m: i64, k: i64, ld_scores: i64, means: *const f64,
                                   scales: *const f64, components: *const f64, ldc: i64, n: i64, out: *mut f64,
                                   row_stride_out: i64) -> c_int;
    pub fn corrla_pca_inverse_f32(ctx: *mut c_void, scores: *const f32, m: i64, k: i64, ld_scores: i64, means: *const f32,
                                   scales: *const f32, components: *const f32, ldc: i64, n: i64, out: *mut f32,
                                   row_stride_out: i64) -> c_int;
    pub fn corrla_pca_inverse_dev_f64(ctx: *mut c_void, scores: *const f64, m: i64, k: i64, ld_scores: i64, means: *const f64,
                                   scales: *const f64, components: *const f64, ldc: i64, n: i64, out: *mut f64,
                                   row_stride_out: i64) -> c_int;
    pub fn corrla_pca_inverse_dev_f32(ctx: *mut c_void, scores: *const f32, m: i64, k: i64, ld_scores: i64, means: *const f32,
                                   scales: *const f32, components: *const f32, ldc: i64, n: i64, out: *mut f32,
                                   row_stride_out: i64) -> c_int;
    pub fn corrla_ctx_last_pca_apply(ctx: *mut c_void, centring_out: *mut c_int, route_out: *mut c_int) -> c_int;
    pub fn corrla_rbf_matrix_f64(ctx: *mut c_void, xq: *const f64, n_q: i64, ldq: i64, xs: *const f64, n_s: i64, lds: i64,
                                  dim: i64, kernel: c_int, eps: f64, out: *mut f64, ld_out: i64) -> c_int;
    pub fn corrla_rbf_matrix_f32(ctx: *mut c_void, xq: *const f32, n_q: i64, ldq: i64, xs: *const f32, n_s: i64, lds: i64,
                                  dim: i64, kernel: c_int, eps: f64, out: *mut f32, ld_out: i64) -> c_int;
    pub fn corrla_rbf_matrix_dev_f64(ctx: *mut c_void, xq: *const f64, n_q: i64, ldq: i64, xs: *const f64, n_s: i64, lds: i64,
                                  dim: i64, kernel: c_int, eps: f64, out: *mut f64, ld_out: i64) -> c_int;
    pub fn corrla_rbf_matrix_dev_f32(ctx: *mut c_void, xq: *const f32, n_q: i64, ldq: i64, xs: *const f32, n_s: i64, lds: i64,
                                  dim: i64, kernel: c_int, eps: f64, out: *mut f32, ld_out: i64) -> c_int;
    pub fn corrla_rbf_apply_f64(ctx: *mut c_void, xq: *const f64, n_q: i64, ldq: i64, xs: *const f64, n_s: i64, lds: i64,
                                 dim: i64, kernel: c_int, eps: f64, poly_degree: c_int, coeffs: *const f64, ldw: i64,
                                 n_rhs: i64, out: *mut f64, ld_out: i64) -> c_int;
    pub fn corrla_rbf_apply_f32(ctx: *mut c_void, xq: *const f32, n_q: i64, ldq: i64, xs: *const f32, n_s: i64, lds: i64,
                                 dim: i64, kernel: c_int, eps: f64, poly_degree: c_int, coeffs: *const f32, ldw: i64,
                                 n_rhs: i64, out: *mut f32, ld_out: i64) -> c_int;
    pub fn corrla_rbf_apply_dev_f64(ctx: *mut c_void, xq: *const f64, n_q: i64, ldq: i64, xs: *const f64, n_s: i64, lds: i64,
                                 dim: i64, kernel: c_int, eps: f64, poly_degree: c_int, coeffs: *const f64, ldw: i64,
                                 n_rhs: i64, out: *mut f64, ld_out: i64) -> c_int;
    pub fn corrla_rbf_apply_dev_f32(ctx: *mut c_void, xq: *const f32, n_q: i64, ldq: i64, xs: *const f32, n_s: i64, lds: i64,
                                 dim: i64, kernel: c_int, eps: f64, poly_degree: c_int, coeffs: *const f32, ldw: i64,
                                 n_rhs: i64, out: *mut f32, ld_out: i64) -> c_int;
}

struct Ctx(*mut c_void);
impl Drop for Ctx {
    fn drop(&mut self) {
        unsafe { corrla_ctx_destroy(self.0) }
    }
}
thread_local! {
    static CTX: Ctx = unsafe {
        let mut c = std::ptr::null_mut();
        check(corrla_ctx_create(0, &mut c));
        Ctx(c)
    };
}

fn check(rc: c_int) {
    if rc != 0 {
        let msg = unsafe { CStr::from_ptr(corrla_last_error()) }.to_string_lossy().into_owned();
        panic!("corrla_rsvd (status {}): {}", rc, msg);
    }
}

pub trait RsvdScalar: faer::Entity + Copy + Default {
    unsafe fn rsvd(ctx: *mut c_void, a: *const Self, m: i64, n: i64, rs: i64, cs: i64, k: i64, q: i64, p: i64,
                   u: *mut Self, ldu: i64, s: *mut Self, vt: *mut Self, ldvt: i64) -> c_int;
    unsafe fn power(ctx: *mut c_void, a: *const Self, m: i64, n: i64, rs: i64, cs: i64, w: i64, q: i64,
                    out: *mut Self, ldq: i64) -> c_int;
}
impl RsvdScalar for f64 {
    unsafe fn rsvd(ctx: *mut c_void, a: *const f64, m: i64, n: i64, rs: i64, cs: i64, k: i64, q: i64, p: i64,
                   u: *mut f64, ldu: i64, s: *mut f64, vt: *mut f64, ldvt: i64) -> c_int {
        corrla_rsvd_f64(ctx, a, m, n, rs, cs, k, q, p, std::ptr::null(), u, ldu, s, vt, ldvt)
    }
    unsafe fn power(ctx: *mut c_void, a: *const f64, m: i64, n: i64, rs: i64, cs: i64, w: i64, q: i64,
                    out: *mut f64, ldq: i64) -> c_int {
        corrla_power_iter_f64(ctx, a, m, n, rs, cs, w, q, std::ptr::null(), out, ldq)
    }
}
impl RsvdScalar for f32 {
    unsafe fn rsvd(ctx: *mut c_void, a: *const f32, m: i64, n: i64, rs: i64, cs: i64, k: i64, q: i64, p: i64,
                   u: *mut f32, ldu: i64, s: *mut f32, vt: *mut f32, ldvt: i64) -> c_int {
        corrla_rsvd_f32(ctx, a, m, n, rs, cs, k, q, p, std::ptr::null(), u, ldu, s, vt, ldvt)
    }
    unsafe fn power(ctx: *mut c_void, a: *const f32, m: i64, n: i64, rs: i64, cs: i64, w: i64, q: i64,
                    out: *mut f32, ldq: i64) -> c_int {
        corrla_power_iter_f32(ctx, a, m, n, rs, cs, w, q, std::ptr::null(), out, ldq)
    }
}

pub fn random_svd<T: RsvdScalar>(a_mat: MatRef<T>, omega_rank: usize, n_iter: usize, n_oversamples: usize)
    -> (Mat<T>, Mat<T>, Mat<T>)
{
    let (m, n, k) = (a_mat.nrows(), a_mat.ncols(), omega_rank);
    let mut u = Mat::<T>::zeros(m, k);
    let mut s = Mat::<T>::zeros(k, 1);
    let mut vt = Mat::<T>::zeros(k, n);
    let rc = CTX.with(|c| unsafe {
        T::rsvd(c.0, a_mat.as_ptr(), m as i64, n as i64, a_mat.row_stride() as i64, a_mat.col_stride() as i64,
                k as i64, n_iter as i64, n_oversamples as i64, u.as_ptr_mut(), u.col_stride() as i64,
                s.as_ptr_mut(), vt.as_ptr_mut(), vt.col_stride() as i64)
    });
    check(rc);
// ... 65 lines not shown
```

Baseline: 93570.

## Add thin-Q kernels for Gram and apply products in RSVD QR

Adds specialised kernels for the skinny Y^T Y Gram and the Y*M apply products used in Cholesky-QR and the final U/V formation. They replace the generic gemm_nn/gemm_tn paths when the planner accepts the shape. The QR can now read straight from the projected matrix, which removes a skinny copy. A plan rejection falls back to the generic GEMM, and the path is on by default through an env knob. The cost is new kernels plus a slab reduction that may or may not beat the tuned generic GEMM at 16k x 128.

New measurement: 94470, median of 6. About the same (+1.0%).

```diff
diff --git a/corrla_rs_amd/_lib.py b/corrla_rs_amd/_lib.py
--- a/corrla_rs_amd/_lib.py
+++ b/corrla_rs_amd/_lib.py
@@ -56,6 +56,7 @@
         "corrla_comm_unique_id": (C.c_int, [vp]),
         "corrla_ctx_comm_init": (C.c_int, [vp, vp, C.c_int, C.c_int]),
         "corrla_ctx_last_pca_apply": (C.c_int, [vp, C.POINTER(C.c_int), C.POINTER(C.c_int)]),
+        "corrla_ctx_last_thinq": (C.c_int, [vp, C.POINTER(C.c_int), C.POINTER(C.c_int), C.POINTER(C.c_int)]),
     }
     for suf, sc in (("f32", flt), ("f64", dbl)):
         rsvd = [vp, vp, i64, i64, i64, i64, i64, i64, i64, C.POINTER(Opts), vp, i64, vp, vp, i64]
@@ -88,6 +89,8 @@
         points = [vp, vp, i64, i64, vp, i64, i64, i64, C.c_int, dbl]
         s["corrla_rbf_matrix_" + suf] = s["corrla_rbf_matrix_dev_" + suf] = (C.c_int, points + [vp, i64])
         s["corrla_rbf_apply_" + suf] = s["corrla_rbf_apply_dev_" + suf] = (C.c_int, points + [C.c_int, vp, i64, i64, vp, i64])
+        s["corrla_thinq_apply_dev_" + suf] = (C.c_int, [vp, vp, i64, i64, i64, vp, i64, i64, vp, C.c_int, vp, i64])
+        s["corrla_thinq_gram_dev_" + suf] = (C.c_int, [vp, vp, i64, i64, i64, vp, i64])
         s["corrla_fill_normal_dev_" + suf] =(C.c_int, [vp, vp, i64, i64, i64, i64, u64, i64, i64])
         s["corrla_time_sketch_dev_" + suf] = (C.c_int, [vp, vp, i64, i64, i64, i64, vp, i64, i64, vp, i64, C.c_int,
                                                          C.POINTER(dbl)])
diff --git a/corrla_rs_amd/api.py b/corrla_rs_amd/api.py
--- a/corrla_rs_amd/api.py
+++ b/corrla_rs_amd/api.py
@@ -655,6 +655,26 @@
         assert x.shape[0] == (m if trans else n) and x.dtype == a.dtype
         return self._run_product("corrla_matmul_", (a, m, n, *a.stride()), m, n, x, trans, beta)
 
+    def thinq_apply(self, y, m, l, ldy, mat, ldm, l2, out, ldo, scale=None, run_if=-1):
+        ct = C.c_float if _suffix(y.dtype) == "f32" else C.c_double
+        sc = C.byref(ct(scale)) if scale is not None else None
+        _sync_stream(y)
+        L.check(self._entry("corrla_thinq_apply_", True, y.dtype)(self._h, y.data_ptr(), m, l, ldy, mat.data_ptr(), ldm, l2, sc,
+                                                                   int(run_if), out.data_ptr(), ldo))
+        return out
+
+    def thinq_gram(self, y, m, l, ldy):
+        import torch
+        g = torch.empty((l, l), dtype=y.dtype, device=y.device)
+        _sync_stream(y)
+        L.check(self._entry("corrla_thinq_gram_", True, y.dtype)(self._h, y.data_ptr(), m, l, ldy, g.data_ptr(), l))
+        return g
+
+    def last_thinq(self):
+        a, g, f = C.c_int(0), C.c_int(0), C.c_int(0)
+        L.check(self._lib.corrla_ctx_last_thinq(self._h, C.byref(a), C.byref(g), C.byref(f)))
+        return a.value, g.value, f.value
+
     def grad_mat(self, x_mat, y, est_order, n_nbrs, x_query=None, *, scale=1.0):
         est_order, n_nbrs = int(est_order), int(n_nbrs)
         nreg = C.c_int(0)
diff --git a/corrla_rs_amd/csrc/capi_impl.hpp b/corrla_rs_amd/csrc/capi_impl.hpp
--- a/corrla_rs_amd/csrc/capi_impl.hpp
+++ b/corrla_rs_amd/csrc/capi_impl.hpp
@@ -474,6 +474,64 @@
       [&] { return stage_input<Dev, T>(dev, false, a, m, n, rs, cs, true); });
 }
 
+template <class Dev, class T>
+inline void thinq_apply_entry(Dev& dev, const T* y, int64_t m, int64_t l, int64_t ldy, const T* mat, int64_t ldm, int64_t l2,
+                              const T* scale, int run_if, T* out, int64_t ldo) {
+  static_assert(dev_has_thinq<Dev>::value, "the thin-Q hooks need a backend with the thin-Q kernels");
+  if (!y || !mat || !out) throw Error(ST_EINVAL, "y, mat or out is NULL");
+  if (m < 1 || l < 1 || l2 < 1) throw Error(ST_EINVAL, "m, l and l2 must be >= 1");
+  if (ldy < m || ldo < m || ldm < l) throw Error(ST_EINVAL, "leading dimension too small");
+  dev.begin_call();
+  T* scale_dev = nullptr;
+  if (scale) {
+    scale_dev = dev.template alloc_scalar<T>(1);
+    dev.store_values(scale, (int64_t)1, scale_dev, false);
+  }
+  int* gate = nullptr;
+  if (run_if >= 0) {
+    gate = dev.alloc_flags(1);
+    const int word = run_if ? 1 : 0;
+    dev.store_values(&word, (int64_t)1, gate, false);
+  }
+  dev.set_run_if(gate);
+  try {
+    const Skinny<T> yv = caller_skinny(const_cast<T*>(y), m, l, ldy);
+    Skinny<T> ms = dev.template alloc_skinny<T>(l, l2);
+    dev.copy_in_skinny(mat, ldm, ms);
+    const bool on_grid = (uintptr_t)mat % 16 == 0 && (ldm * sizeof(T)) % 16 == 0;
+    const Skinny<T> mv = on_grid ? ms : caller_skinny(const_cast<T*>(mat), l, l2, ldm);
+    Skinny<T> ov = caller_skinny(out, m, l2, ldo);
+    if (!dev.thinq_apply(yv, l, mv, ov, (const T*)scale_dev)) {
+      Skinny<T> ys = dev.template alloc_skinny<T>(m, l), os = dev.template alloc_skinny<T>(m, l2);
+      dev.copy_in_skinny(y, ldy, ys);
+      dev.gemm_tn(as_rowmajor_transposed(ys, l), ms, os, (const T*)scale_dev);
+      if (run_if != 0) dev.copy_out(os, l2, out, ldo, false, false);
+    }
+  } catch (...) {
+    dev.set_run_if(nullptr);
+    throw;
+  }
+  dev.set_run_if(nullptr);
+  dev.end_call();
+}
+
+template <class Dev, class T>
+inline void thinq_gram_entry(Dev& dev, const T* y, int64_t m, int64_t l, int64_t ldy, T* g, int64_t ldg) {
+  static_assert(dev_has_thinq<Dev>::value, "the thin-Q hooks need a backend with the thin-Q kernels");
+  if (!y || !g) throw Error(ST_EINVAL, "y or g is NULL");
+  if (m < 1 || l < 1) throw Error(ST_EINVAL, "m and l must be >= 1");
+  if (ldy < m || ldg < l) throw Error(ST_EINVAL, "leading dimension too small");
+  dev.begin_call();
+  Skinny<T> ys = dev.template alloc_skinny<T>(m, l), gs = dev.template alloc_skinny<T>(l, l);
+  dev.copy_in_skinny(y, ldy, ys);
+  if (!dev.thinq_gram(ys, l, gs)) {
+    Skinny<T> yv = ys.view_cols(l);
+    dev.gemm_nn(as_rowmajor_transposed(ys, l), yv, gs, (const T*)nullptr);
+  }
+  dev.copy_out(gs, l, g, ldg, false, false);
+  dev.end_call();
+}
+
 inline void validate_csr_args(const void* values, const void* ci, const void* rp, int64_t m, int64_t n, int64_t nnz) {
   if (!values || !ci || !rp) throw Error(ST_EINVAL, "values, col_idx or row_ptr is NULL");
   if (m < 1 || n < 1) throw Error(ST_EINVAL, "matrix must have at least one row and one column");
diff --git a/corrla_rs_amd/csrc/corrla_rsvd.hip b/corrla_rs_amd/csrc/corrla_rsvd.hip
--- a/corrla_rs_amd/csrc/corrla_rsvd.hip
+++ b/corrla_rs_amd/csrc/corrla_rsvd.hip
@@ -9,6 +9,7 @@
 #include "pca_apply_stage.hpp"
 #include "rbf_stage.hpp"
 #include "tall_stage.hpp"
+#include "thinq_stage.hpp"
 
 using namespace corrla;
 
@@ -331,6 +332,31 @@
     std::lock_guard<std::mutex> lk(c->mu);
     if (centring_out) *centring_out = c->pca_apply.centring;
     if (route_out) *route_out = c->pca_apply.route;
+  });
+}
+
+#define CORRLA_DEFINE_THINQ(SUF, T)                                                                                     \
+  CORRLA_API corrla_status corrla_thinq_apply_dev_##SUF(corrla_ctx* ctx, const T* y, int64_t m, int64_t l, int64_t ldy,  \
+                                                        const T* mat, int64_t ldm, int64_t l2, const T* scale, int run_if, \
+                                                        T* out, int64_t ldo) {                                          \
+    return ctx_call(ctx, [&](corrla_ctx& c) {                                                                           \
+      thinq_apply_entry<HipDev, T>(c.dev, y, m, l, ldy, mat, ldm, l2, scale, run_if, out, ldo);                          \
+    });                                                                                                                 \
+  }                                                                                                                     \
+  CORRLA_API corrla_status corrla_thinq_gram_dev_##SUF(corrla_ctx* ctx, const T* y, int64_t m, int64_t l, int64_t ldy, T* g, \
+                                                       int64_t ldg) {                                                   \
+    return ctx_call(ctx, [&](corrla_ctx& c) { thinq_gram_entry<HipDev, T>(c.dev, y, m, l, ldy, g, ldg); });              \
+  }
+CORRLA_DEFINE_THINQ(f32, float)
+CORRLA_DEFINE_THINQ(f64, double)
+CORRLA_API corrla_status corrla_ctx_last_thinq(corrla_ctx* ctx, int* n_apply_out, int* n_gram_out, int* n_fallback_out) {
+  return guarded([&] {
+    corrla_ctx* c = need(ctx);
+    std::lock_guard<std::mutex> lk(c->mu);
+    const HipDev::ThinqRan& r = c->dev.thinq_ran();
+    if (n_apply_out) *n_apply_out = r.apply;
+    if (n_gram_out) *n_gram_out = r.gram;
+    if (n_fallback_out) *n_fallback_out = r.fallback;
   });
 }
 
diff --git a/corrla_rs_amd/csrc/driver.hpp b/corrla_rs_amd/csrc/driver.hpp
--- a/corrla_rs_amd/csrc/driver.hpp
+++ b/corrla_rs_amd/csrc/driver.hpp
@@ -95,6 +95,11 @@
 struct dev_has_rbf : std::false_type {};
 template <class D>
 struct dev_has_rbf<D, std::void_t<decltype(D::kHasRbf)>> : std::true_type {};
+
+template <class D, class = void>
+struct dev_has_thinq : std::false_type {};
+template <class D>
+struct dev_has_thinq<D, std::void_t<decltype(D::kHasThinq)>> : std::true_type {};
 
 template <class T>
 struct TallA {
@@ -346,16 +351,17 @@
     }
   }
 
-  int64_t orthonormalize(Skinny<T>& y, Skinny<T>& tmp, bool sharded, bool rough = false) {
+  int64_t orthonormalize(Skinny<T>& y, Skinny<T>& tmp, bool sharded, bool rough = false, const Skinny<T>* src = nullptr) {
     const int64_t l = y.cols;
     if (householder_usable(y, sharded)) {
+      if (src) dev.copy_skinny(*src, y);
       PhaseTimer qt0;
       householder_thin_q_any_width(y, tmp, sharded);
       ++tm.qr_passes;
       subphase(tm.qr_gram_ms, qt0);
       return l;
     }
-    int64_t r = orthonormalize_core(y, tmp, sharded, rough);
+    int64_t r = orthonormalize_core(y, tmp, sharded, rough, false, src);
     if (r < l && !att_.defer && (sharded ? global_rows(true) : y.rows) >= l) r = complete_basis(y, r, sharded);
     return r;
   }
@@ -380,17 +386,41 @@
     return r + rc;
   }
 
+  void gram_product(const Skinny<T>& y, int64_t l, Skinny<T>& g) {
+    if constexpr (dev_has_thinq<Dev>::value)
+      if (dev.thinq_gram(y, l, g)) return;
+    Skinny<T> yv = y.view_cols(l);
+    dev.gemm_nn(as_rowmajor_transposed(y, l), yv, g, kNone);
+  }
+  void apply_product(const Skinny<T>& y, int64_t l, const Skinny<T>& mat, Skinny<T>& out) {
+    if constexpr (dev_has_thinq<Dev>::value)
+      if (dev.thinq_apply(y, l, mat, out, kNone)) return;
+    dev.gemm_tn(as_rowmajor_transposed(y, l), mat, out, kNone);
+  }
+
   template <class Factor>
-  void cholqr_pass(Skinny<T>& y, Skinny<T>& tmp, Skinny<T>& gd, bool sharded, bool inplace, Factor&& factor) {
+  void cholqr_pass(Skinny<T>& y, Skinny<T>& tmp, Skinny<T>& gd, bool sharded, bool inplace, Factor&& factor,
+                   const Skinny<T>* src = nullptr) {
     const int64_t l = y.cols;
-    Skinny<T> yv = y.view_cols(l);
-    dev.gemm_nn(as_rowmajor_transposed(y, l), yv, gd, kNone);
+    const Skinny<T>& in = src ? *src : y;
+    gram_product(in, l, gd);
     if (sharded) dev.allreduce(gd.p, (size_t)gd.ld * (size_t)gd.cols_alloc);
     const Skinny<T> md = factor(gd);
     if (inplace) {
-      dev.apply_inplace(y, l, md);
+      if constexpr (dev_has_thinq<Dev>::value) {
+        Skinny<T> out = y.view_cols(l);
+        Skinny<T> mv = md.view_cols(l);
+        mv.rows = l;
+        if (dev.thinq_apply(in, l, mv, out, kNone)) return;
+      }
+      if (src) {
+        Skinny<T> out = y.view_cols(l);
+        dev.gemm_tn(as_rowmajor_transposed(in, l), md, out, kNone);
+      } else {
+        dev.apply_inplace(y, l, md);
+      }
     } else {
-      dev.gemm_tn(as_rowmajor_transposed(y, l), md, tmp, kNone);
+      apply_product(in, l, md, tmp);
       std::swap(y.p, tmp.p);
     }
   }
@@ -430,7 +460,8 @@
     dev.copy_block(x22, 0, 0, n2, n2, md, n1, n1);
   }
 
-  int64_t orthonormalize_device(Skinny<T>& y, Skinny<T>& tmp, bool sharded, bool rough, bool polish) {
+  int64_t orthonormalize_device(Skinny<T>& y, Skinny<T>& tmp, bool sharded, bool rough, bool polish,
+                                const Skinny<T>* src = nullptr) {
     const int64_t l = y.cols;
     PhaseTimer qt0;
     const bool inplace = dev.qr_inplace_fits(l);
@@ -473,7 +504,7 @@
         });
         dev.template combine_need<T>(need + pass, need_ratio > 0.f ? nullptr : insp, need_blk, need_blk + 1);
         return md;
-      });
+      }, pass == 0 ? src : nullptr);
       if (pass + 1 < npass || inloop)
         dev.refill_null(y, l, null_mask, (uint64_t)(0x9e3779b97f4a7c15ull ^ (uint64_t)(977 * (att_.flags_used + pass) + l)));
       if (pass < always) ++tm.qr_passes;
@@ -485,12 +516,14 @@
     return l;
   }
 
-  int64_t orthonormalize_core(Skinny<T>& y, Skinny<T>& tmp, bool sharded, bool rough, bool polish = false) {
+  int64_t orthonormalize_core(Skinny<T>& y, Skinny<T>& tmp, bool sharded, bool rough, bool polish = false,
+                              const Skinny<T>* src = nullptr) {
     const int64_t l = y.cols;
     int64_t r = l;
     if (att_.defer && (sharded || y.rows >= l) && att_.flags_used + kRobustPasses <= att_.flags_cap &&
         dev.template device_qr_robust_fits<T>(l))
-      return orthonormalize_device(y, tmp, sharded, rough, polish);
+      return orthonormalize_device(y, tmp, sharded, rough, polish, src);
+    if (src) dev.copy_skinny(*src, y);
     const int rpp = dev.template device_chol_fits<T>(l) ? 1 : (dev.template device_chol_blocked_fits<T>(l) ? 2 : 0);
     if (rpp > 0) {
       PhaseTimer qt0;
@@ -833,8 +866,11 @@
     phase(tm.project_ms, pt);
     Skinny<T> qb = dev.template alloc_skinny<T>(a.nt, l);
     Skinny<T> qb2 = dev.template alloc_skinny<T>(a.nt, l);
-    dev.copy_skinny(bt, qb);
-    orthonormalize(qb, qb2, false);
+    const Skinny<T>* qb_src = nullptr;
+    if constexpr (dev_has_thinq<Dev>::value)
+      if (dev.thinq_enabled()) qb_src = &bt;
+    if (!qb_src) dev.copy_skinny(bt, qb);
+    orthonormalize(qb, qb2, false, false, qb_src);
     phase(tm.qr_ms, pt);
     Skinny<T> ct = dev.template alloc_skinny<T>(l, l);
     dev.gemm_nn(as_rowmajor_transposed(bt, l), qb, ct, kNone);
@@ -865,9 +901,9 @@
       }
     }
     phase(tm.small_svd_ms, pt);
-    dev.gemm_tn(as_rowmajor_transposed(qb, l), m2, v_tall, kNone);
+    apply_product(qb, l, m2, v_tall);
     dev.fix_signs(v_tall, m1, k);
-    dev.gemm_tn(as_rowmajor_transposed(q, l), m1, u_tall, kNone);
+    apply_product(q, l, m1, u_tall);
     phase(tm.finalize_ms, pt);
     tm.host_enqueue_ms += total.lap();
   }
diff --git a/corrla_rs_amd/csrc/hip_backend.hpp b/corrla_rs_amd/csrc/hip_backend.hpp
--- a/corrla_rs_amd/csrc/hip_backend.hpp
+++ b/corrla_rs_amd/csrc/hip_backend.hpp
@@ -106,6 +106,10 @@
 template <class T>
 void set_lds_limits();
 }
+namespace thinq_stage {
+template <class T>
+void set_lds_limits();
+}
 
 class HipDev {
  public:
@@ -155,6 +159,7 @@
     gemm_knobs_.no_rotate = env_int("CORRLA_GEMM_NO_ROTATE", 0) != 0;
     gemm_knobs_.mixed_split = env_int("CORRLA_MIXED_SPLIT", 0);
     syrk_knobs_.slab_rows = env_int("CORRLA_SYRK_SLAB_ROWS", 0);
+    thinq_kernels_ = env_int("CORRLA_THINQ_KERNELS", 1) != 0;
   }
   ~HipDev() {
     (void)hipSetDevice(device);
@@ -210,6 +215,7 @@
     events_set_[0] = events_set_[1] = events_set_[2] = false;
     n_collectives = 0;
     collective_bytes = 0;
+    thinq_ran_ = ThinqRan();
     marks_.clear();
     ev_used_ = 0;
     phase_mark(nullptr);
@@ -328,6 +334,17 @@
   void gemm_nn(const Big<T>& r, const Skinny<T>& x, Skinny<T>& out, const T* scale_dev);
   template <class T>
   void gemm_tn(const Big<T>& r, const Skinny<T>& x, Skinny<T>& out, const T* scale_dev);
+
+  static constexpr bool kHasThinq = true;
+  bool thinq_enabled() const { return thinq_kernels_; }
+  template <class T>
+  bool thinq_apply(const Skinny<T>& y, int64_t l, const Skinny<T>& mat, Skinny<T>& out, const T* scale_dev);
+  template <class T>
+  bool thinq_gram(const Skinny<T>& y, int64_t l, Skinny<T>& g);
+  struct ThinqRan {
+    int apply = 0, gram = 0, fallback = 0;
+  };
+  const ThinqRan& thinq_ran() const { return thinq_ran_; }
 
   static constexpr bool kHasSpmm = true;
   template <class T>
@@ -1060,6 +1077,8 @@
   int gemm_debug_flags_ = 0;
   GemmKnobs gemm_knobs_;
   SyrkKnobs syrk_knobs_;
+  bool thinq_kernels_ = true;
+  ThinqRan thinq_ran_;
   uint64_t entropy_ = 0, calls_ = 0, calls_sharded_ = 0;
   bool no_device_chol_ = false;
   const int* run_if_ = nullptr;
@@ -1101,6 +1120,7 @@
   static void set_lds_limits_typed() {
     constexpr size_t kMax = k::kLdsMaxBytes;
     tall_stage::set_lds_limits<T>();
+    thinq_stage::set_lds_limits<T>();
     rbf_stage::set_lds_limits<T>();
     lds_limit((const void*)k::syrk_kernel<T, true>, (size_t)k::syrk_lds_bytes((int)sizeof(T)));
     lds_limit((const void*)k::syrk_kernel<T, false>, (size_t)k::syrk_lds_bytes((int)sizeof(T)));
diff --git a/corrla_rs_amd/csrc/thinq_kernels.hpp b/corrla_rs_amd/csrc/thinq_kernels.hpp
--- /dev/null
+++ b/corrla_rs_amd/csrc/thinq_kernels.hpp
@@ -0,0 +1,229 @@
+#pragma once
+#include "tall_kernels.hpp"
+#include "thinq_plan.hpp"
+
+namespace corrla {
+namespace k {
+
+template <class T>
+struct ThinqApplyArgs {
+  const T* y;
+  int64_t m, ld_y;
+  int kdim;
+  const T* mat;
+  int64_t ld_m;
+  int n2;
+  T* out;
+  int64_t ld_o;
+  int out_cols;
+  const T* scale;
+  int vec_store;
+  int dma_mat;
+  int64_t row_blocks;
+  const T* zero;
+  const int* run_if;
+};
+
+template <class T, int NT>
+__global__ __launch_bounds__(256) void thinq_apply_kernel(ThinqApplyArgs<T> g) {
+  typedef typename MT<T>::vec_t vec_t;
+  typedef typename MT<T>::acc_t acc_t;
+  constexpr int VEC = MT<T>::VEC;
+  constexpr int NKS = 4 * NT;
+  constexpr int NJV = NKS / VEC;
+  extern __shared__ __attribute__((aligned(16))) char smem[];
+  if (g.run_if && *g.run_if == 0) return;
+  T* bl = (T*)smem;
+  const int lane = threadIdx.x & 63;
+  const int wave = __builtin_amdgcn_readfirstlane(threadIdx.x >> 6);
+  const int fi = lane & 15, kq = lane >> 4;
+  const int njv = (g.kdim + 4 * VEC - 1) / (4 * VEC);
+
+  const int trow = sizeof(T) == 4 ? fi : 4 * (fi & 3) + (fi >> 2);
+  T a[NKS];
+  auto load_rows = [&](int64_t blk) {
+    const int64_t row = blk * kThinqApplyRows + 16 * wave + trow;
+    const T* src = g.y + (int64_t)(VEC * kq) * g.ld_y + row;
+#pragma unroll
+    for (int j = 0; j < NKS; ++j) {
+      const int kk = 4 * VEC * (j / VEC) + (j % VEC);
+      a[j] = (T)0;
+      if (j / VEC < njv && kk + VEC * kq < g.kdim && row < g.m) a[j] = src[(int64_t)kk * g.ld_y];
+    }
+  };
+  load_rows(blockIdx.x);
+
+  if (g.dma_mat) {
+    for (int pc = wave; pc < NT * njv; pc += 4) {
+      const int ct = pc / njv, jv = pc - ct * njv;
+      const int col = 16 * ct + fi, kk = 4 * VEC * jv + VEC * kq;
+      const T* src = (col < g.n2 && kk < g.kdim) ? g.mat + (int64_t)col * g.ld_m + kk : g.zero;
+      glds16(src, (char*)bl + (ct * NJV + jv) * 1024);
+    }
+    wait_vmcnt<0>();
+  } else {
+    for (int pc = wave; pc < NT * njv; pc += 4) {
+      const int ct = pc / njv, jv = pc - ct * njv;
+      const int col = 16 * ct + fi, kk = 4 * VEC * jv + VEC * kq;
+      vec_t v;
+#pragma unroll
+      for (int e = 0; e < VEC; ++e) v[e] = (col < g.n2 && kk + e < g.kdim) ? g.mat[(int64_t)col * g.ld_m + kk + e] : (T)0;
+      *(vec_t*)(bl + ((ct * NJV + jv) * 64 + lane) * VEC) = v;
+    }
+  }
+  __syncthreads();
+  const T sc = g.scale ? *g.scale : (T)1;
+
+  for (int64_t blk = blockIdx.x; blk < g.row_blocks; blk += gridDim.x) {
+    const int64_t r0 = blk * kThinqApplyRows + 16 * wave;
+    acc_t acc[NT];
+#pragma unroll
+    for (int ct = 0; ct < NT; ++ct) acc[ct] = (acc_t){0, 0, 0, 0};
+#pragma unroll
+    for (int jv = 0; jv < NJV; ++jv) {
+      if (jv < njv) {
+        vec_t b[NT];
+#pragma unroll
+        for (int ct = 0; ct < NT; ++ct) b[ct] = *(const vec_t*)(bl + ((ct * NJV + jv) * 64 + lane) * VEC);
+#pragma unroll
+        for (int e = 0; e < VEC; ++e)
+#pragma unroll
+          for (int ct = 0; ct < NT; ++ct) acc[ct] = MT<T>::mma(a[jv * VEC + e], b[ct][e], acc[ct]);
+      }
+    }
+    const int64_t row = r0 + 4 * kq;
+#pragma unroll
+    for (int ct = 0; ct < NT; ++ct) {
+      const int col = 16 * ct + fi;
+      if (col < g.out_cols) {
+        T* dst = g.out + (int64_t)col * g.ld_o + row;
+        if (g.vec_store && row + 3 < g.m) {
+#pragma unroll
+          for (int h = 0; h < 4 / VEC; ++h) {
+            vec_t w;
+#pragma unroll
+            for (int e = 0; e < VEC; ++e) w[e] = acc[ct][h * VEC + e] * sc;
+            *(vec_t*)(dst + h * VEC) = w;
+          }
+        } else {
+#pragma unroll
+          for (int jp = 0; jp < 4; ++jp)
+            if (row + jp < g.m) dst[jp] = acc[ct][jp] * sc;
+        }
+      }
+    }
+    if (blk + gridDim.x < g.row_blocks) load_rows(blk + gridDim.x);
+  }
+}
+
+template <class T, int NCT, int Z>
+__device__ __forceinline__ void thinq_gram_run(const TallGramArgs<T>& g, char* smem) {
+  typedef typename MT<T>::vec_t vec_t;
+  typedef typename MT<T>::acc_t acc_t;
+  constexpr int VEC = MT<T>::VEC;
+  constexpr int ROWS = gram_rows<T>();
+  constexpr int TILE = gram_tile_bytes(NCT);
+  constexpr int NS = gram_stages(NCT);
+  static_assert(NS >= 2, "ring too shallow");
+  constexpr int NPAIR = thinq_gram_pairs(NCT), CH = thinq_gram_chunk(NCT);
+  constexpr int P0 = Z * CH, P1 = (Z + 1) * CH < NPAIR ? (Z + 1) * CH : NPAIR;
+  constexpr int A0 = thinq_gram_pair_row(NCT, P0);
+  constexpr int NCHUNK = 8 * NCT;
+  constexpr int DPL = NCHUNK / 4 - 2 * A0;
+  const int lane = threadIdx.x & 63;
+  const int wave = __builtin_amdgcn_readfirstlane(threadIdx.x >> 6);
+  const int fi = lane & 15, kq = lane >> 4;
+  const int64_t rows = (g.m + VEC - 1) / VEC * VEC;
+  const int64_t r_begin = (int64_t)blockIdx.x * g.rows_per_group;
+  const int64_t r_end = min(rows, r_begin + g.rows_per_group);
+  const int ntile = r_begin < r_end ? (int)((r_end - r_begin + ROWS - 1) / ROWS) : 0;
+
+  auto stage = [&](int buf, int t) {
+    char* rt = smem + buf * TILE;
+    const int64_t row0 = r_begin + (int64_t)t * ROWS;
+#pragma unroll
+    for (int i = 2 * A0; i < NCHUNK / 4; ++i) {
+      const int ch = wave + 4 * i;
+      const int c = 2 * ch + (lane >> 5);
+      const int ps = lane & 31;
+      const int q = (ps & 16) | ((ps ^ c) & 15);
+      const int64_t row = row0 + VEC * q;
+      const T* src = (row < r_end && c < g.l) ? g.y + (int64_t)c * g.ld + row : g.zero;
+      glds16(src, rt + ch * 1024);
+    }
+  };
+  for (int t = 0; t < NS - 1 && t < ntile; ++t) stage(t % NS, t);
+
+  acc_t acc[P1 - P0];
+#pragma unroll
+  for (int p = 0; p < P1 - P0; ++p) acc[p] = (acc_t){0, 0, 0, 0};
+
+  for (int t = 0; t < ntile; ++t) {
+    if (t + NS - 2 < ntile)
+      wait_vmcnt<(NS - 2) * DPL>();
+    else
+      wait_vmcnt<0>();
+    wg_barrier();
+    if (t + NS - 1 < ntile) stage((t + NS - 1) % NS, t + NS - 1);
+    const char* tb = smem + (t % NS) * TILE;
+#pragma unroll
+    for (int s = 0; s < 2; ++s) {
+      const int q = 8 * wave + 4 * s + kq;
+      vec_t fr[NCT];
+#pragma unroll
+      for (int a = A0; a < NCT; ++a) {
+        const int c = 16 * a + fi;
+        fr[a] = *(const vec_t*)(tb + c * 512 + (((q & 16) | ((q ^ c) & 15)) << 4));
+      }
+#pragma unroll
+      for (int e = 0; e < VEC; ++e) {
+        int p = 0;
+#pragma unroll
+        for (int a = 0; a < NCT; ++a)
+#pragma unroll
+          for (int b = a; b < NCT; ++b, ++p)
+            if (p >= P0 && p < P1) acc[p - P0] = MT<T>::mma(fr[a][e], fr[b][e], acc[p - P0]);
+      }
+    }
+  }
+  __syncthreads();
+  T* red = (T*)smem;
+  if (wave > 0) {
+#pragma unroll
+    for (int p = 0; p < P1 - P0; ++p)
+#pragma unroll
+      for (int j = 0; j < 4; ++j) red[((wave - 1) * CH + p) * 256 + j * 64 + lane] = acc[p][j];
+  }
+  __syncthreads();
+  if (wave == 0) {
+    T* dst = g.slab + (int64_t)blockIdx.x * g.slab_stride;
+    int p = 0;
+#pragma unroll
+    for (int a = 0; a < NCT; ++a)
+#pragma unroll
+      for (int b = a; b < NCT; ++b, ++p)
+        if (p >= P0 && p < P1) {
+#pragma unroll
+          for (int j = 0; j < 4; ++j) {
+            const int o = (p - P0) * 256 + j * 64 + lane;
+            const T v = ((acc[p - P0][j] + red[o]) + red[CH * 256 + o]) + red[2 * CH * 256 + o];
+            const int gr = 16 * a + MT<T>::drow(lane, j), gc = 16 * b + fi;
+            dst[(int64_t)gc * g.out_ld + gr] = v;
+            if (a != b) dst[(int64_t)gr * g.out_ld + gc] = v;
+          }
+        }
+  }
+}
+
+template <class T, int NCT>
+__global__ __launch_bounds__(256) void thinq_gram_kernel(TallGramArgs<T> g) {
+  extern __shared__ __attribute__((aligned(16))) char smem[];
+  if (g.run_if && *g.run_if == 0) return;
+  const int z = __builtin_amdgcn_readfirstlane(blockIdx.y);
+  static_for<0, thinq_gram_nz(NCT)>([&](auto zc) {
+    if (z == decltype(zc)::value) thinq_gram_run<T, NCT, decltype(zc)::value>(g, smem);
+  });
+}
+
+}
+}
diff --git a/corrla_rs_amd/csrc/thinq_plan.hpp b/corrla_rs_amd/csrc/thinq_plan.hpp
--- /dev/null
+++ b/corrla_rs_amd/csrc/thinq_plan.hpp
@@ -0,0 +1,140 @@
+#pragma once
+#include "gemm_plan.hpp"
+
+namespace corrla {
+
+constexpr int kThinqMaxTiles = 9;
+
+namespace k {
+
+constexpr int kThinqApplyRows = 64;
+CORRLA_HD constexpr int thinq_apply_lds_bytes(int nt, int esz) { return 4 * nt * nt * 64 * esz; }
+CORRLA_HD constexpr int thinq_apply_max_tiles(int esz) {
+  int nt = kThinqMaxTiles;
+  while (nt > 1 && thinq_apply_lds_bytes(nt, esz) > (int)kLdsMaxBytes) --nt;
+  return nt;
+}
+
+CORRLA_HD constexpr int thinq_gram_pairs(int nct) { return nct * (nct + 1) / 2; }
+CORRLA_HD constexpr int thinq_gram_chunk(int nct) { return (thinq_gram_pairs(nct) + 3) / 4; }
+CORRLA_HD constexpr int thinq_gram_nz(int nct) { return (thinq_gram_pairs(nct) + thinq_gram_chunk(nct) - 1) / thinq_gram_chunk(nct); }
+CORRLA_HD constexpr int thinq_gram_pair_row(int nct, int p) {
+  int a = 0;
+  while (a < nct - 1 && p >= nct - a) {
+    p -= nct - a;
+    ++a;
+  }
+  return a;
+}
+CORRLA_HD constexpr int thinq_gram_lds_bytes(int nct, int esz) {
+  const int ring = gram_stages(nct) * gram_tile_bytes(nct);
+  const int red = 3 * thinq_gram_chunk(nct) * 256 * esz;
+  return ring > red ? ring : red;
+}
+constexpr int kThinqGramMaxGroups = 64;
+
+}
+
+struct ThinqApplyShape {
+  int esz = 4;
+  GemmOperand y, mat, out;
+  bool inplace = false;
+  int num_cus = 256;
+};
+struct ThinqApplyPlan {
+  const char* reject = nullptr;
+  int nt = 0;
+  unsigned grid = 0;
+  int block = 256;
+  int rows_per_wg = k::kThinqApplyRows;
+  int64_t row_blocks = 0;
+  int lds = 0;
+  int nks = 0;
+  int64_t out_cols = 0;
+  int vec_store = 0;
+  int dma_mat = 0;
+};
+
+inline ThinqApplyPlan thinq_apply_plan(const ThinqApplyShape& s, const GemmKnobs& kn) {
+  ThinqApplyPlan p;
+  auto no = [&](const char* why) {
+    p.reject = why;
+    return p;
+  };
+  if (s.esz != 4 && s.esz != 8) return no("element type");
+  const int64_t m = s.y.rows, l = s.y.cols, l2 = s.mat.cols;
+  const int vec = k::gemm_vec(s.esz);
+  const int max_l = 16 * k::thinq_apply_max_tiles(s.esz);
+  if (m < 1 || l < 1 || l2 < 1) return no("empty product");
+  if (l > max_l || l2 > max_l) return no("M does not fit in LDS");
+  if (s.mat.rows != l) return no("inner dimensions differ");
+  const int tall_l = 16 * tall_max_tiles(s.esz);
+  if (kn.tall_min_rows > 0 && m >= kn.tall_min_rows && l <= tall_l && l2 <= tall_l) return no("the tall kernels serve");
+  if (s.y.ld < m || s.out.ld < m || s.mat.ld < l) return no("leading dimension below the row count");
+  if (s.out.rows != m || s.out.cols < l2) return no("output shape");
+  if (s.inplace && s.out.ld != s.y.ld) return no("in place with another leading dimension");
+  const int nct2 = (int)((l2 + 15) / 16);
+  p.out_cols = std::min<int64_t>(s.out.external ? s.out.cols : s.out.cols_alloc, 16 * nct2);
+  if (p.out_cols < l2) return no("output shape");
+  p.nt = (int)std::max((l + 15) / 16, (l2 + 15) / 16);
+  p.nks = (int)((l + 3) / 4);
+  p.lds = k::thinq_apply_lds_bytes(p.nt, s.esz);
+  p.row_blocks = (m + p.rows_per_wg - 1) / p.rows_per_wg;
+  const int per_cu = std::max(1, std::min(4, (int)k::kLdsMaxBytes / p.lds));
+  p.grid = (unsigned)std::min<int64_t>(p.row_blocks, (int64_t)s.num_cus * per_cu);
+  p.vec_store = (s.out.aligned && s.out.ld % vec == 0) ? 1 : 0;
+  p.dma_mat = (!s.mat.external && s.mat.aligned && s.mat.ld % vec == 0 && s.mat.ld >= (l + 3) / 4 * 4) ? 1 : 0;
+  return p;
+}
+
+struct ThinqGramShape {
+  int esz = 4;
+  GemmOperand y, out;
+  int num_cus = 256;
+  int max_slabs = k::kThinqGramMaxGroups;
+};
+struct ThinqGramPlan {
+  const char* reject = nullptr;
+  int nct = 0;
+  unsigned grid[2] = {0, 0};
+  int block = 256;
+  int rows_tile = 0;
+  int64_t rows_per_group = 0, groups = 0;
+  int lds = 0;
+  int64_t slab_stride = 0;
+  size_t slab_bytes = 0;
+  SlabReducePlan reduce;
+};
+
+inline ThinqGramPlan thinq_gram_plan(const ThinqGramShape& s, const GemmKnobs& kn) {
+  ThinqGramPlan p;
+  auto no = [&](const char* why) {
+    p.reject = why;
+    return p;
+  };
+  if (s.esz != 4 && s.esz != 8) return no("element type");
+  const int64_t m = s.y.rows, l = s.y.cols;
+  const int vec = k::gemm_vec(s.esz);
+  if (m < 1 || l < 1) return no("empty product");
+  if (l > 16 * kThinqMaxTiles) return no("more than one column block");
+  if (kn.tall_min_rows > 0 && m >= kn.tall_min_rows && l <= 16 * tall_max_tiles(s.esz)) return no("the tall kernels serve");
+  if (s.y.external || s.out.external) return no("operands without zero padding");
+  if (!s.y.aligned || s.y.ld % vec != 0 || s.y.ld < (m + vec - 1) / vec * vec) return no("16-byte pieces of a column not addressable");
+  p.nct = (int)((l + 15) / 16);
+  if (s.out.ld < 16 * p.nct || s.out.cols_alloc < 16 * p.nct) return no("output padding below the column tiles");
+  p.rows_tile = s.esz == 4 ? k::gram_rows<float>() : k::gram_rows<double>();
+  const int64_t tiles = (m + p.rows_tile - 1) / p.rows_tile;
+  const int64_t cap = std::max(1, std::min(k::kThinqGramMaxGroups, s.max_slabs));
+  const int64_t tiles_per_group = (tiles + cap - 1) / cap;
+  p.rows_per_group = tiles_per_group * p.rows_tile;
+  p.groups = (tiles + tiles_per_group - 1) / tiles_per_group;
+  p.grid[0] = (unsigned)p.groups;
+  p.grid[1] = (unsigned)k::thinq_gram_nz(p.nct);
+  p.lds = k::thinq_gram_lds_bytes(p.nct, s.esz);
+  p.slab_stride = s.out.ld * s.out.cols_alloc;
+  p.slab_bytes = (size_t)p.groups * (size_t)p.slab_stride * s.esz;
+  p.reduce = {SlabReduce::deep, {(unsigned)((l + 63) / 64), (unsigned)(16 * p.nct)}, (int)p.groups, l, 16 * p.nct};
+  return p;
+}
+
+}
diff --git a/corrla_rs_amd/csrc/thinq_stage.hpp b/corrla_rs_amd/csrc/thinq_stage.hpp
--- /dev/null
+++ b/corrla_rs_amd/csrc/thinq_stage.hpp
@@ -0,0 +1,93 @@
+#pragma once
+#include "tall_stage.hpp"
+#include "thinq_kernels.hpp"
+
+namespace corrla {
+namespace thinq_stage {
+
+template <class T>
+inline void set_lds_limits() {
+  for_each_nt<k::thinq_apply_max_tiles((int)sizeof(T))>([](auto nt) {
+    lds_limit((const void*)k::thinq_apply_kernel<T, decltype(nt)::value>, k::thinq_apply_lds_bytes(nt, (int)sizeof(T)));
+  });
+  for_each_nt<kThinqMaxTiles>([](auto nct) {
+    lds_limit((const void*)k::thinq_gram_kernel<T, decltype(nct)::value>, k::thinq_gram_lds_bytes(nct, (int)sizeof(T)));
+  });
+}
+
+template <class T>
+inline GemmOperand operand(const Skinny<T>& x) {
+  return {x.rows, x.cols, x.ld, 0, x.cols_alloc, x.external, (uintptr_t)x.p % 16 == 0};
+}
+
+template <class T>
+inline void apply(const tall_stage::Call& c, const ThinqApplyPlan& p, const Skinny<T>& y, const Skinny<T>& mat, Skinny<T>& out,
+                  const T* scale_dev) {
+  const k::ThinqApplyArgs<T> g{y.p,   y.rows, y.ld,           (int)y.cols, mat.p,       mat.ld,    (int)mat.cols,
+                               out.p, out.ld, (int)p.out_cols, scale_dev,   p.vec_store, p.dma_mat, p.row_blocks,
+                               (const T*)c.zero_page, c.run_if};
+  with_nt<k::thinq_apply_max_tiles((int)sizeof(T))>(p.nt, [&](auto nt) {
+    hipLaunchKernelGGL((k::thinq_apply_kernel<T, decltype(nt)::value>), dim3(p.grid), dim3(p.block), p.lds, c.stream, g);
+  });
+  CORRLA_HIP(hipGetLastError());
+}
+
+template <class T>
+inline void gram(const tall_stage::Call& c, const ThinqGramPlan& p, const Skinny<T>& y, Skinny<T>& out) {
+  T* slab = (T*)c.dev.alloc_bytes(p.slab_bytes);
+  const k::TallGramArgs<T> g{y.p, y.rows, y.ld, (int)y.cols, slab, p.slab_stride, out.ld, p.rows_per_group, (const T*)c.zero_page,
+                             c.run_if};
+  with_nt<kThinqMaxTiles>(p.nct, [&](auto nct) {
+    hipLaunchKernelGGL((k::thinq_gram_kernel<T, decltype(nct)::value>), dim3(p.grid[0], p.grid[1]), dim3(p.block), p.lds, c.stream, g);
+  });
+  CORRLA_HIP(hipGetLastError());
+  tall_stage::slab_reduce<T>(c, p.reduce, slab, p.slab_stride, out.p, out.ld, (const T*)nullptr, c.run_if);
+}
+
+}
+
+template <class T>
+bool HipDev::thinq_apply(const Skinny<T>& y, int64_t l, const Skinny<T>& mat, Skinny<T>& out, const T* scale_dev) {
+  if (!thinq_kernels_) return false;
+  Skinny<T> yv = y.view_cols(l);
+  Skinny<T> mv = mat;
+  mv.rows = l;
+  ThinqApplyShape s;
+  s.esz = (int)sizeof(T);
+  s.y = thinq_stage::operand(yv);
+  s.mat = thinq_stage::operand(mv);
+  s.out = thinq_stage::operand(out);
+  s.inplace = (const void*)out.p == (const void*)y.p;
+  s.num_cus = num_cus;
+  const ThinqApplyPlan p = thinq_apply_plan(s, gemm_knobs_);
+  if (p.reject) {
+    ++thinq_ran_.fallback;
+    return false;
+  }
+  thinq_stage::apply(tall_call(), p, yv, mv, out, scale_dev);
+  ++thinq_ran_.apply;
+  return true;
+}
+
+template <class T>
+bool HipDev::thinq_gram(const Skinny<T>& y, int64_t l, Skinny<T>& g) {
+  if (!thinq_kernels_) return false;
+  Skinny<T> yv = y.view_cols(l);
+  ThinqGramShape s;
+  s.esz = (int)sizeof(T);
+  s.y = thinq_stage::operand(yv);
+  s.out = thinq_stage::operand(g);
+  s.num_cus = num_cus;
+  const GemmPlan today = gemm_plan(tall_stage::shape(false, as_rowmajor_transposed(y, l), yv, g, 0, num_cus), gemm_knobs_);
+  if (!today.error) s.max_slabs = std::max(1, today.nsplit);
+  const ThinqGramPlan p = thinq_gram_plan(s, gemm_knobs_);
+  if (p.reject) {
+    ++thinq_ran_.fallback;
+    return false;
+  }
+  thinq_stage::gram(tall_call(), p, yv, g);
+  ++thinq_ran_.gram;
+  return true;
+}
+
+}
diff --git a/include/corrla_rsvd.h b/include/corrla_rsvd.h
--- a/include/corrla_rsvd.h
+++ b/include/corrla_rsvd.h
@@ -291,6 +291,18 @@
                                                  const double* xq, int64_t n_q, int est_order, int64_t n_nbrs,
                                                  double out_scale, double* g, int64_t ldg, int* n_regularised);
 
+CORRLA_API corrla_status corrla_thinq_apply_dev_f32(corrla_ctx* ctx, const float* y, int64_t m, int64_t l, int64_t ldy,
+                                                    const float* mat, int64_t ldm, int64_t l2, const float* scale, int run_if,
+                                                    float* out, int64_t ldo);
+CORRLA_API corrla_status corrla_thinq_apply_dev_f64(corrla_ctx* ctx, const double* y, int64_t m, int64_t l, int64_t ldy,
+                                                    const double* mat, int64_t ldm, int64_t l2, const double* scale, int run_if,
+                                                    double* out, int64_t ldo);
+CORRLA_API corrla_status corrla_thinq_gram_dev_f32(corrla_ctx* ctx, const float* y, int64_t m, int64_t l, int64_t ldy, float* g,
+                                                   int64_t ldg);
+CORRLA_API corrla_status corrla_thinq_gram_dev_f64(corrla_ctx* ctx, const double* y, int64_t m, int64_t l, int64_t ldy, double* g,
+                                                   int64_t ldg);
+CORRLA_API corrla_status corrla_ctx_last_thinq(corrla_ctx* ctx, int* n_apply_out, int* n_gram_out, int* n_fallback_out);
+
 CORRLA_API corrla_status corrla_time_sketch_dev_f32(corrla_ctx* ctx, const float* a, int64_t m, int64_t n, int64_t row_stride,
                                          int64_t col_stride, const float* x, int64_t ldx, int64_t l, float* y,
                                          int64_t ldy, int reps, double* avg_ms);
diff --git a/integration/rust/src/lib.rs b/integration/rust/src/lib.rs
--- a/integration/rust/src/lib.rs
+++ b/integration/rust/src/lib.rs
@@ -130,6 +130,14 @@
                                    scales: *const f32, components: *const f32, ldc: i64, n: i64, out: *mut f32,
                                    row_stride_out: i64) -> c_int;
     pub fn corrla_ctx_last_pca_apply(ctx: *mut c_void, centring_out: *mut c_int, route_out: *mut c_int) -> c_int;
+    pub fn corrla_thinq_apply_dev_f64(ctx: *mut c_void, y: *const f64, m: i64, l: i64, ldy: i64, mat: *const f64, ldm: i64,
+                                       l2: i64, scale: *const f64, run_if: c_int, out: *mut f64, ldo: i64) -> c_int;
+    pub fn corrla_thinq_apply_dev_f32(ctx: *mut c_void, y: *const f32, m: i64, l: i64, ldy: i64, mat: *const f32, ldm: i64,
+                                       l2: i64, scale: *const f32, run_if: c_int, out: *mut f32, ldo: i64) -> c_int;
+    pub fn corrla_thinq_gram_dev_f64(ctx: *mut c_void, y: *const f64, m: i64, l: i64, ldy: i64, g: *mut f64, ldg: i64) -> c_int;
+    pub fn corrla_thinq_gram_dev_f32(ctx: *mut c_void, y: *const f32, m: i64, l: i64, ldy: i64, g: *mut f32, ldg: i64) -> c_int;
+    pub fn corrla_ctx_last_thinq(ctx: *mut c_void, n_apply_out: *mut c_int, n_gram_out: *mut c_int,
+                                 n_fallback_out: *mut c_int) -> c_int;
     pub fn corrla_rbf_matrix_f64(ctx: *mut c_void, xq: *const f64, n_q: i64, ldq: i64, xs: *const f64, n_s: i64, lds: i64,
                                   dim: i64, kernel: c_int, eps: f64, out: *mut f64, ld_out: i64) -> c_int;
     pub fn corrla_rbf_matrix_f32(ctx: *mut c_void, xq: *const f32, n_q: i64, ldq: i64, xs: *const f32, n_s: i64, lds: i64,
```
